# gwall-ceres/HighRes-net

Hardware: AMD Instinct MI355X
Metric: SR frames/sec (384x384 out) at B=32, n_views=32 (higher is better)
Workload: dtype bf16

## Files before the change

### highres-net_amd/hrnet_hip/csrc/api.hip

```cpp
#include "../../../include/hrnet_hip.h"
#include "kernels.h"
#include "hrnet_layout.h"
#include "shiftnet_layout.h"

#include <stdarg.h>
#include <stdio.h>
#include <stdlib.h>
#include <string.h>

static thread_local char g_err[512] = "";
void hrn_set_error(const char* fmt, ...) {
    va_list ap;
    va_start(ap, fmt);
    vsnprintf(g_err, sizeof g_err, fmt, ap);
    va_end(ap);
}

namespace {

using namespace hrn;

struct HrnetWs {
    size_t ref, emb, buf_a, buf_b, fused, total;
};
HrnetWs hrnet_ws(int dt, int B, int V, int H, int W) {
    HrnetWs w;
    const size_t es = hrn_esize(dt), hw = (size_t)H * W;
    const size_t stack = (size_t)B * V * hw * 64 * es;
    size_t off = 0;
    auto take = [&](size_t bytes) { size_t o = off; off = hrn_align_up(off + bytes, ALIGN); return o; };
    w.ref = take((size_t)B * hw * 4);
    w.emb = take(stack);
    w.buf_a = take(stack);
    w.buf_b = take(stack);
    w.fused = take((size_t)B * hw * 64 * es);
    w.total = off;
    return w;
}

size_t stack_lo(int dt, int B, int V, int H, int W) { return dt == HRN_BF16X3 ? (size_t)B * V * H * W * 64 * 2 : 0; }
size_t fused_lo(int dt, int B, int H, int W) { return dt == HRN_BF16X3 ? (size_t)B * H * W * 64 * 2 : 0; }
bool dtype_ok(int dt) { return dt == HRN_F32 || dt == HRN_BF16 || dt == HRN_BF16X3; }

int check_scale(int scale) {
    HRN_CHECK(hrn_scale_ok(scale), -2, "scale must be 2, 3 or 4 (decoder kernel_size == stride; got %d)", scale);
    return 0;
}

int check_common(int dt, int nl, int B, int V, int H, int W) {
    HRN_CHECK(dtype_ok(dt), -2, "dtype must be HRN_DTYPE_F32, HRN_DTYPE_BF16 or HRN_DTYPE_BF16X3 (got %d)", dt);
    HRN_CHECK(nl >= 0 && nl <= HRN_MAX_RES_LAYERS, -2, "num_layers %d out of range 0..%d", nl, HRN_MAX_RES_LAYERS);
    HRN_CHECK(B > 0 && V > 0 && H > 0 && W > 0, -2, "empty input B=%d V=%d H=%d W=%d", B, V, H, W);
    return 0;
}

int encoder_impl(const void* pk, int dt, int nl, const float* lrs, int B, int V, int H, int W,
                 void* emb, void* ws, const HrnetWs& wl, hipStream_t s) {
    const HrnetLayout L = hrnet_layout(dt, nl, 3);
    const size_t hw = (size_t)H * W;
    float* ref = (float*)at(ws, wl.ref);
    void* bufA = at(ws, wl.buf_a);
    void* bufB = at(ws, wl.buf_b);
    int rc;
    if ((rc = hrn_launch_median(lrs, ref, B, V, H, W, s))) return rc;
    const size_t lo = stack_lo(dt, B, V, H, W);
    if ((rc = hrn_launch_stem(dt, lrs, hw, ref, V, hw, nullptr, (const float*)at(pk, L.stem_w), (const float*)at(pk, L.stem_b),
                              (const float*)at(pk, L.stem_a), bufA, B * V, H, W, s, lo))) return rc;
    for (int l = 0; l < nl; ++l) {
        ConvParams p = conv_base(B * V, H, W);
        p.in = bufA; p.out = bufB; p.in_lo = p.out_lo = lo;
        p.wpk = at(pk, L.enc_w[2 * l]); p.bias = (const float*)at(pk, L.enc_b[2 * l]); p.slope = (const float*)at(pk, L.enc_a[2 * l]);
        if ((rc = hrn_launch_conv3x3(dt, 64, 64, p, s, false))) return rc;
        ConvParams q = conv_base(B * V, H, W);
        q.in = bufB; q.out = bufA; q.res = bufA; q.res_mode = 1; q.in_lo = q.out_lo = q.res_lo = lo;
        q.wpk = at(pk, L.enc_w[2 * l + 1]); q.bias = (const float*)at(pk, L.enc_b[2 * l + 1]); q.slope = (const float*)at(pk, L.enc_a[2 * l + 1]);
        if ((rc = hrn_launch_conv3x3(dt, 64, 64, q, s, false))) return rc;
    }
    ConvParams f = conv_base(B * V, H, W);
    f.in = bufA; f.out = emb; f.in_lo = f.out_lo = lo;
    f.wpk = at(pk, L.encf_w); f.bias = (const float*)at(pk, L.encf_b); f.slope = nullptr;
    return hrn_launch_conv3x3(dt, 64, 64, f, s, false);
}

int fuse_impl(const void* pk, int dt, int nl, int alpha_residual, void* emb, const float* alphas, int B, int V, int H, int W,
              void* fused, void* ws, const HrnetWs& wl, hipStream_t s) {
    const HrnetLayout L = hrnet_layout(dt, nl, 3);
    const size_t hw = (size_t)H * W, es = hrn_esize(dt);
    void* t1 = at(ws, wl.buf_a);
    void* t2 = at(ws, wl.buf_b);
    const size_t lo = stack_lo(dt, B, V, H, W), flo = fused_lo(dt, B, H, W);
    int n = V, rc;
    if (n / 2 == 0) {
        HRN_HIP(hipMemcpyAsync(fused, emb, (size_t)B * hw * 64 * es, hipMemcpyDeviceToDevice, s));
        return 0;
    }
    while (n / 2 > 0) {
        const int parity = n & 1, half = n >> 1;
        const bool last = (half == 1);
        ConvParams a = conv_base(B * half, H, W);
        a.in_pair = 1; a.stack = emb; a.pair_h = half; a.pair_last = n - parity - 1; a.pair_vs = V;
        a.out = t1; a.stack_lo = a.out_lo = lo;
        a.wpk = at(pk, L.fres_w[0]); a.bias = (const float*)at(pk, L.fres_b[0]); a.slope = (const float*)at(pk, L.fres_a[0]);
        if ((rc = hrn_launch_conv3x3(dt, 128, 128, a, s, false))) return rc;
        ConvParams b = conv_base(B * half, H, W);
        b.in = t1; b.out = t2; b.in_lo = b.out_lo = b.stack_lo = lo;
        b.res_mode = 2;
        b.stack = emb; b.pair_h = half; b.pair_last = n - parity - 1; b.pair_vs = V;
        b.wpk = at(pk, L.fres_w[1]); b.bias = (const float*)at(pk, L.fres_b[1]); b.slope = (const float*)at(pk, L.fres_a[1]);
        if ((rc = hrn_launch_conv3x3(dt, 128, 128, b, s, false))) return rc;
        ConvParams c = conv_base(B * half, H, W);
        c.in = t2; c.in_lo = c.res_lo = lo;
        c.out_h = half;
        if (last) { c.out = fused; c.out_vs = 1; c.out_lo = flo; } else { c.out = emb; c.out_vs = V; c.out_lo = lo; }
        c.pair_last = n - parity - 1;
        if (alpha_residual) { c.res_mode = 3; c.res = emb; c.res_vs = V; c.alphas = alphas; c.alpha_vs = V; }
        c.wpk = at(pk, L.fout_w); c.bias = (const float*)at(pk, L.fout_b); c.slope = (const float*)at(pk, L.fout_a);
        if ((rc = hrn_launch_conv3x3(dt, 128, 64, c, s, false))) return rc;
        n = half;
    }
    return 0;
}

int decoder_impl(const void* pk, int dt, int nl, int scale, const void* fused, int N, int H, int W, float* sr, hipStream_t s) {
    const HrnetLayout L = hrnet_layout(dt, nl, scale);
    return hrn_launch_decoder(dt, fused, at(pk, L.dec_w), (const float*)at(pk, L.dec_b), (const float*)at(pk, L.dec_a),
                              (const float*)at(pk, L.fin_w), (const float*)at(pk, L.fin_b), sr, N, H, W, s, fused_lo(dt, N, H, W), scale);
}

struct SnWs {
    size_t means, scale, shift, partial, x, y, fc, xr, fc_partial, total;
};
SnWs sn_ws(int B) {
    SnWs w;
    size_t off = 0;
    auto take = [&](size_t bytes) { size_t o = off; off = hrn_align_up(off + bytes, ALIGN); return o; };
    w.means = take((size_t)B * 2 * 4);
    w.scale = take(128 * 4); w.shift = take(128 * 4);
    w.partial = take((size_t)SN_PARTIAL_BLOCKS * 128 * 2 * 8);
    w.x = take((size_t)B * 128 * 128 * 64 * 4);
    w.y = take((size_t)B * 128 * 128 * 64 * 4);
    w.fc = take((size_t)B * 1024 * 4);
    w.xr = take((size_t)B * 32768 * 4);
    w.fc_partial = take(hrn_fc1_partial_bytes());
    w.total = off;
    return w;
}

}

extern "C" {

int hrn_version(void) { return HRN_ABI_VERSION; }
const char* hrn_last_error(void) { return g_err; }

size_t hrn_hrnet_packed_bytes_s(int dtype, int num_layers, int scale) {
    if (!dtype_ok(dtype) || num_layers < 0 || num_layers > HRN_MAX_RES_LAYERS || !hrn_scale_ok(scale)) return 0;
    return hrnet_layout(dtype, num_layers, scale).total;
}

int hrn_hrnet_pack_s(const hrn_hrnet_params* P, int dt, int scale, void* packed, size_t packed_bytes, void* stream) {
    int rc;
    if ((rc = check_scale(scale))) return rc;
    HRN_CHECK(P && packed, -2, "hrn_hrnet_pack: null argument");
    if ((rc = check_common(dt, P->num_layers, 1, 1, 1, 1))) return rc;
    const int nl = P->num_layers;
    const HrnetLayout L = hrnet_layout(dt, nl, scale);
    HRN_CHECK(packed_bytes >= L.total, -3, "hrn_hrnet_pack: packed buffer too small (%zu < %zu)", packed_bytes, L.total);
    hipStream_t s = (hipStream_t)stream;
    auto copy = [&](size_t off, const float* src, size_t n) -> int {
        HRN_CHECK(src != nullptr, -2, "hrn_hrnet_pack: null parameter pointer");
        HRN_HIP(hipMemcpyAsync(at(packed, off), src, n * 4, hipMemcpyDeviceToDevice, s));
        return 0;
    };
    if ((rc = copy(L.stem_w, P->enc_init_w, 64 * 18)) || (rc = copy(L.stem_b, P->enc_init_b, 64)) || (rc = copy(L.stem_a, P->enc_init_a, 1))) return rc;
    for (int i = 0; i < 2 * nl; ++i) {
        HRN_CHECK(P->enc_res_w[i], -2, "hrn_hrnet_pack: null encoder weight %d", i);
        if ((rc = hrn_launch_conv_pack(dt, 64, 64, P->enc_res_w[i], at(packed, L.enc_w[i]), s))) return rc;
        if ((rc = copy(L.enc_b[i], P->enc_res_b[i], 64)) || (rc = copy(L.enc_a[i], P->enc_res_a[i], 1))) return rc;
    }
    HRN_CHECK(P->enc_final_w && P->fuse_out_w && P->dec_w, -2, "hrn_hrnet_pack: null weight pointer");
    if ((rc = hrn_launch_conv_pack(dt, 64, 64, P->enc_final_w, at(packed, L.encf_w), s))) return rc;
    if ((rc = copy(L.encf_b, P->enc_final_b, 64))) return rc;
    for (int i = 0; i < 2; ++i) {
        HRN_CHECK(P->fuse_res_w[i], -2, "hrn_hrnet_pack: null fuse weight %d", i);
        if ((rc = hrn_launch_conv_pack(dt, 128, 128, P->fuse_res_w[i], at(packed, L.fres_w[i]), s))) return rc;
        if ((rc = copy(L.fres_b[i], P->fuse_res_b[i], 128)) || (rc = copy(L.fres_a[i], P->fuse_res_a[i], 1))) return rc;
    }
    if ((rc = hrn_launch_conv_pack(dt, 128, 64, P->fuse_out_w, at(packed, L.fout_w), s))) return rc;
    if ((rc = copy(L.fout_b, P->fuse_out_b, 64)) || (rc = copy(L.fout_a, P->fuse_out_a, 1))) return rc;
    if ((rc = hrn_launch_decoder_pack(dt == HRN_BF16X3 ? HRN_F32 : dt, P->dec_w, at(packed, L.dec_w), s, scale))) return rc;
    if ((rc = copy(L.dec_b, P->dec_b, 64)) || (rc = copy(L.dec_a, P->dec_a, 1))) return rc;
    if ((rc = copy(L.fin_w, P->fin_w, 64)) || (rc = copy(L.fin_b, P->fin_b, 1))) return rc;
    return 0;
}

size_t hrn_hrnet_workspace_bytes(int dtype, int B, int V, int H, int W) {
    if (!dtype_ok(dtype) || B <= 0 || V <= 0 || H <= 0 || W <= 0) return 0;
    return hrnet_ws(dtype, B, V, H, W).total;
}

int hrn_encoder_forward(const void* packed, int dt, int nl, const float* lrs, int B, int V, int H, int W,
                        void* emb, void* ws, size_t ws_bytes, void* stream) {
    int rc;
    if ((rc = check_common(dt, nl, B, V, H, W))) return rc;
    HRN_CHECK(packed && lrs && emb && ws, -2, "hrn_encoder_forward: null argument");
    const HrnetWs wl = hrnet_ws(dt, B, V, H, W);
    HRN_CHECK(ws_bytes >= wl.total, -3, "hrn_encoder_forward: workspace too small (%zu < %zu)", ws_bytes, wl.total);
    return encoder_impl(packed, dt, nl, lrs, B, V, H, W, emb, ws, wl, (hipStream_t)stream);
}

int hrn_fuse_forward(const void* packed, int dt, int nl, int alpha_residual, void* emb, const float* alphas,
                     int B, int V, int H, int W, void* fused, void* ws, size_t ws_bytes, void* stream) {
    int rc;
    if ((rc = check_common(dt, nl, B, V, H, W))) return rc;
    HRN_CHECK(packed && emb && alphas && fused && ws, -2, "hrn_fuse_forward: null argument");
    const HrnetWs wl = hrnet_ws(dt, B, V, H, W);
    HRN_CHECK(ws_bytes >= wl.total, -3, "hrn_fuse_forward: workspace too small (%zu < %zu)", ws_bytes, wl.total);
    return fuse_impl(packed, dt, nl, alpha_residual, emb, alphas, B, V, H, W, fused, ws, wl, (hipStream_t)stream);
}

int hrn_decoder_forward_s(const void* packed, int dt, int nl, int scale, const void* fused, int N, int H, int W, float* sr, void* stream) {
    int rc;
    if ((rc = check_scale(scale)) || (rc = check_common(dt, nl, N, 1, H, W))) return rc;
    HRN_CHECK(packed && fused && sr, -2, "hrn_decoder_forward: null argument");
    return decoder_impl(packed, dt, nl, scale, fused, N, H, W, sr, (hipStream_t)stream);
}

int hrn_hrnet_forward_s(const void* packed, int dt, int nl, int scale, int alpha_residual, const float* lrs, const float* alphas,
                        int B, int V, int H, int W, float* sr, void* ws, size_t ws_bytes, void* stream) {
    int rc;
    if ((rc = check_scale(scale)) || (rc = check_common(dt, nl, B, V, H, W))) return rc;
    HRN_CHECK(packed && lrs && alphas && sr && ws, -2, "hrn_hrnet_forward: null argument");
    const HrnetWs wl = hrnet_ws(dt, B, V, H, W);
    HRN_CHECK(ws_bytes >= wl.total, -3, "hrn_hrnet_forward: workspace too small (%zu < %zu)", ws_bytes, wl.total);
    hipStream_t s = (hipStream_t)stream;
    void* emb = at(ws, wl.emb);
    void* fused = at(ws, wl.fused);
    if ((rc = encoder_impl(packed, dt, nl, lrs, B, V, H, W, emb, ws, wl, s))) return rc;
    if ((rc = fuse_impl(packed, dt, nl, alpha_residual, emb, alphas, B, V, H, W, fused, ws, wl, s))) return rc;
    return decoder_impl(packed, dt, nl, scale, fused, B, H, W, sr, s);
}

size_t hrn_shiftnet_packed_bytes(void) { return sn_layout().total; }

int hrn_shiftnet_pack(const hrn_shiftnet_params* P, void* packed, size_t packed_bytes, void* stream) {
    HRN_CHECK(P && packed, -2, "hrn_shiftnet_pack: null argument");
    const SnLayout L = sn_layout();
    HRN_CHECK(packed_bytes >= L.total, -3, "hrn_shiftnet_pack: packed buffer too small (%zu < %zu)", packed_bytes, L.total);
    hipStream_t s = (hipStream_t)stream;
    int rc;
    for (int i = 0; i < 8; ++i) {
        HRN_CHECK(P->conv_w[i] && P->conv_b[i], -2, "hrn_shiftnet_pack: null conv parameter %d", i);
        if (i == 0) {
            HRN_HIP(hipMemcpyAsync(at(packed, L.conv_w[0]), P->conv_w[0], 64 * 18 * 4, hipMemcpyDeviceToDevice, s));
        } else if ((rc = hrn_launch_conv_pack(HRN_F32, SN_CI[i], SN_CO[i], P->conv_w[i], at(packed, L.conv_w[i]), s))) {
            return rc;
        }
        HRN_HIP(hipMemcpyAsync(at(packed, L.conv_b[i]), P->conv_b[i], SN_CO[i] * 4, hipMemcpyDeviceToDevice, s));
    }
    HRN_CHECK(P->fc1_b && P->fc2_w, -2, "hrn_shiftnet_pack: null fc parameter");
    HRN_HIP(hipMemcpyAsync(at(packed, L.fc1_b), P->fc1_b, 1024 * 4, hipMemcpyDeviceToDevice, s));
    HRN_HIP(hipMemcpyAsync(at(packed, L.fc2_w), P->fc2_w, 2 * 1024 * 4, hipMemcpyDeviceToDevice, s));
    return 0;
}

size_t hrn_shiftnet_workspace_bytes(int B) { return B > 0 ? sn_ws(B).total : 0; }

int hrn_shiftnet_forward(const void* packed, const hrn_shiftnet_params* P, const float* x, int B, int train_bn, float momentum,
                         const unsigned char* dropout_mask, float* theta, void* ws, size_t ws_bytes, void* stream) {
    HRN_CHECK(packed && P && x && theta && ws, -2, "hrn_shiftnet_forward: null argument");
    HRN_CHECK(P->fc1_w, -2, "hrn_shiftnet_forward: params->fc1_w is null (fc1.weight is read in place)");
    HRN_CHECK(B > 0, -2, "hrn_shiftnet_forward: empty batch");
    const SnLayout L = sn_layout();
    const SnWs wl = sn_ws(B);
    HRN_CHECK(ws_bytes >= wl.total, -3, "hrn_shiftnet_forward: workspace too small (%zu < %zu)", ws_bytes, wl.total);
    hipStream_t s = (hipStream_t)stream;
    float* means = (float*)at(ws, wl.means);
    float* scale = (float*)at(ws, wl.scale);
    float* shift = (float*)at(ws, wl.shift);
    double* partial = (double*)at(ws, wl.partial);
    float* bx = (float*)at(ws, wl.x);
    float* by = (float*)at(ws, wl.y);
    float* fc = (float*)at(ws, wl.fc);
    int rc, hsz = 128;
    const size_t plane = 128 * 128;
    if ((rc = hrn_launch_plane_mean(x, means, B * 2, plane, s))) return rc;
    for (int i = 0; i < 8; ++i) {
        HRN_CHECK(P->bn_g[i] && P->bn_b[i] && P->bn_rm[i] && P->bn_rv[i], -2, "hrn_shiftnet_forward: null BatchNorm tensor %d", i);
        const int C = SN_CO[i];
        if (i > 0 && !train_bn) {
            if ((rc = hrn_launch_bn_fold(P->bn_g[i], P->bn_b[i], P->bn_rm[i], P->bn_rv[i], 1e-5f, (const float*)at(packed, L.conv_b[i]),
                                         scale, shift, C, s))) return rc;
            ConvParams p = conv_base(B, hsz, hsz);
            p.in = by; p.out = bx;
            p.wpk = at(packed, L.conv_w[i]); p.scale = scale; p.bias = shift; p.relu = 1;
            if ((rc = hrn_launch_conv3x3(HRN_F32, SN_CI[i], C, p, s, false))) return rc;
            if (SN_POOL[i]) {
                if ((rc = hrn_launch_bn_act_pool(HRN_F32, bx, nullptr, nullptr, by, B, hsz, hsz, C, 1, s))) return rc;
                hsz /= 2;
            } else {
                float* t = bx; bx = by; by = t;
            }
            continue;
        }
        if (i == 0) {
            if ((rc = hrn_launch_stem(HRN_F32, x, 2 * plane, x + plane, 1, 2 * plane, means, (const float*)at(packed, L.conv_w[0]),
                                      (const float*)at(packed, L.conv_b[0]), nullptr, bx, B, hsz, hsz, s, 0))) return rc;
        } else {
            ConvParams p = conv_base(B, hsz, hsz);
            p.in = by; p.out = bx;
            p.wpk = at(packed, L.conv_w[i]); p.bias = (const float*)at(packed, L.conv_b[i]);
            if ((rc = hrn_launch_conv3x3(HRN_F32, SN_CI[i], SN_CO[i], p, s, false))) return rc;
        }
        if (train_bn) {
            if ((rc = hrn_launch_bn_stats(HRN_F32, bx, (size_t)B * hsz * hsz, C, P->bn_g[i], P->bn_b[i], 1e-5f, scale, shift,
                                          P->bn_rm[i], P->bn_rv[i], momentum, partial, SN_PARTIAL_BLOCKS, s))) return rc;
        } else {
            if ((rc = hrn_launch_bn_fold(P->bn_g[i], P->bn_b[i], P->bn_rm[i], P->bn_rv[i], 1e-5f, nullptr, scale, shift, C, s))) return rc;
        }
        if ((rc = hrn_launch_bn_act_pool(HRN_F32, bx, scale, shift, by, B, hsz, hsz, C, SN_POOL[i], s))) return rc;
        if (SN_POOL[i]) hsz /= 2;
    }
    float* xr = (float*)at(ws, wl.xr);
    if ((rc = hrn_launch_fc_to_ref(HRN_F32, by, dropout_mask, xr, B, s))) return rc;
    if ((rc = hrn_launch_fc1(xr, P->fc1_w, (const float*)at(packed, L.fc1_b), fc, B, (float*)at(ws, wl.fc_partial), s))) return rc;
    return hrn_launch_fc2(fc, (const float*)at(packed, L.fc2_w), theta, B, s);
}

int hrn_lanczos_kernel(const float* dx, int n, float* taps, void* stream) {
    HRN_CHECK(n >= 0 && (n == 0 || (dx && taps)), -2, "hrn_lanczos_kernel: bad argument");
    return hrn_launch_lanczos_taps(dx, n, taps, (hipStream_t)stream);
}

int hrn_lanczos_shift(const float* img, const float* shift, int b, int c, int H, int W, float* out, void* stream) {
    HRN_CHECK(b >= 0 && c >= 0 && H > 0 && W > 0, -2, "hrn_lanczos_shift: bad shape");
    HRN_CHECK(b * c == 0 || (img && shift && out), -2, "hrn_lanczos_shift: null argument");
    return hrn_launch_lanczos_shift(img, shift, b, c, H, W, out, (hipStream_t)stream);
}

size_t hrn_lanczos_shift_backward_workspace_bytes(int b, int c, int H, int W) {
    if (b <= 0 || c <= 0 || H <= 0 || W <= 0) return 0;
    return hrn_lanczos_bwd_workspace_bytes_impl(b, c, H, W);
}

int hrn_lanczos_shift_backward(const float* img, const float* shift, const float* d_out, int b, int c, int H, int W, float* d_img,
                               float* d_shift, void* ws, size_t ws_bytes, void* stream) {
    HRN_CHECK(img && shift && d_out && ws, -2, "hrn_lanczos_shift_backward: null argument");
    HRN_CHECK(b > 0 && c > 0, -2, "hrn_lanczos_shift_backward: empty input b=%d c=%d", b, c);
    HRN_CHECK(ws_bytes >= hrn_lanczos_bwd_workspace_bytes_impl(b, c, H, W), -3, "hrn_lanczos_shift_backward: workspace too small");
    return hrn_launch_lanczos_shift_bwd(img, shift, d_out, b, c, H, W, d_img, d_shift, ws, (hipStream_t)stream);
}

int hrn_get_loss(const float* srs, const float* hrs, const float* maps, int B, int S, int crop, int metric, float* out, void* stream) {
    HRN_CHECK(B > 0 && S > 0 && crop >= 0 && 2 * crop < S, -2, "hrn_get_loss: bad shape B=%d S=%d crop=%d", B, S, crop);
    HRN_CHECK(metric >= 0 && metric <= 2, -2, "hrn_get_loss: metric must be 0 (masked_MSE), 1 (cMSE) or 2 (cPSNR)");
    HRN_CHECK(srs && hrs && maps && out, -2, "hrn_get_loss: null argument");
    return hrn_launch_masked_cmse(srs, hrs, maps, B, S, crop, metric, out, (hipStream_t)stream);
}

size_t hrn_get_loss_train_workspace_bytes(int B) { return B > 0 ? hrn_loss_train_workspace_bytes_impl(B) : 0; }

int hrn_get_loss_train(const float* srs, const float* hrs, const float* maps, int B, int S, int crop, int metric, float* out,
                       double* stats, void* ws, size_t ws_bytes, void* stream) {
    HRN_CHECK(B > 0 && B <= 65535 && S > 0 && crop >= 0 && 2 * crop < S, -2, "hrn_get_loss_train: bad shape B=%d S=%d crop=%d", B, S, crop);
    HRN_CHECK(metric == 1 || metric == 2, -2, "hrn_get_loss_train: metric must be 1 (cMSE) or 2 (cPSNR); masked_MSE has no registered form");
    HRN_CHECK(srs && hrs && maps && out && stats && ws, -2, "hrn_get_loss_train: null argument");
    HRN_CHECK(ws_bytes >= hrn_loss_train_workspace_bytes_impl(B), -3, "hrn_get_loss_train: workspace too small");
    return hrn_launch_loss_train(srs, hrs, maps, B, S, crop, metric, out, stats, (double*)ws, (hipStream_t)stream);
}

int hrn_get_loss_backward(const float* srs, const float* hrs, const float* maps, const double* stats, const float* d_out, int B, int S,
                          int crop, int metric, float* d_srs, void* stream) {
    HRN_CHECK(B > 0 && B <= 65535 && S > 0 && crop >= 0 && 2 * crop < S, -2, "hrn_get_loss_backward: bad shape B=%d S=%d crop=%d", B, S, crop);
    HRN_CHECK(metric == 1 || metric == 2, -2, "hrn_get_loss_backward: metric must be 1 (cMSE) or 2 (cPSNR)");
    HRN_CHECK(srs && hrs && maps && stats && d_out && d_srs, -2, "hrn_get_loss_backward: null argument");
    return hrn_launch_loss_backward(srs, hrs, maps, stats, d_out, B, S, crop, metric, d_srs, (hipStream_t)stream);
}

size_t hrn_shift_cpsnr_workspace_bytes(int B, int border) {
    if (B <= 0 || border < 0) return 0;
    return (size_t)B * (2 * border + 1) * (2 * border + 1) * sizeof(double);
}

int hrn_shift_cpsnr(const float* srs, const float* hrs, const float* maps, int B, int S, int border, int clip, float* out,
                    void* ws, size_t ws_bytes, void* stream) {
    HRN_CHECK(B > 0 && border >= 0 && S > 2 * border, -2, "hrn_shift_cpsnr: bad shape B=%d S=%d border=%d", B, S, border);
    HRN_CHECK(B <= 65535, -2, "hrn_shift_cpsnr: batch %d exceeds the grid limit", B);
    HRN_CHECK(srs && hrs && maps && out && ws, -2, "hrn_shift_cpsnr: null argument");
    HRN_CHECK(ws_bytes >= hrn_shift_cpsnr_workspace_bytes(B, border), -3, "hrn_shift_cpsnr: workspace too small");
    return hrn_launch_shift_cpsnr(srs, hrs, maps, B, S, border, clip, (double*)ws, out, (hipStream_t)stream);
}

}
```

### highres-net_amd/hrnet_hip/csrc/conv3x3.h

```cpp
#pragma once
#include "common.h"

#define CONV_TILE_H 8
#define CONV_TILE_W 32
#define CONV_STEP_BYTES 8192

struct ConvParams {
    const void* in;
    const void* stack;
    int in_pair;
    void* out;
    const void* res;
    const float* alphas;
    const void* wpk;
    const float* bias;
    const float* slope;
    int M, H, W;
    int pair_h, pair_last, pair_vs;
    int out_h, out_vs;
    int res_mode;
    int alpha_vs, res_vs;
    int relu;
    const float* scale;
    size_t in_lo, stack_lo, out_lo, res_lo;
    const float* only_if_nonpos;
};

static inline size_t conv_packed_elems(int cin, int cout) { return (size_t)cin * cout * 9; }

int hrn_launch_conv3x3(int dt, int cin, int cout, const ConvParams& p, hipStream_t stream, bool general_only);

int hrn_launch_conv3x3_r64(const ConvParams& p, hipStream_t stream);

int hrn_launch_conv3x3_v6(int cin, int cout, const ConvParams& p, hipStream_t stream);

int hrn_launch_conv3x3_v6x3(int cin, int cout, const ConvParams& p, hipStream_t stream);

int hrn_launch_conv_pack(int dt, int cin, int cout, const float* w_oihw, void* packed, hipStream_t stream);
```

### highres-net_amd/hrnet_hip/csrc/conv3x3.hip

```cpp
#include "conv3x3.h"
#include <stdlib.h>


namespace {

constexpr int HALO_H = CONV_TILE_H + 2;
constexpr int HALO_W = CONV_TILE_W + 2;
constexpr int PIX_PITCH = 144;
constexpr int IN_LDS_BYTES = HALO_H * HALO_W * PIX_PITCH;
constexpr int W_ROW_PITCH = 144;
constexpr int N_IN_CHUNKS16 = HALO_H * HALO_W * 8;

struct TileCtx {
    int m, y0, x0;
    const unsigned char* src0;
    const unsigned char* src1;
    const unsigned char* in_plain;
};

template <int DT, int CIN, int COUT>
__global__ __launch_bounds__(256 * (COUT / 64), 2) void conv3x3_kernel(const ConvParams p) {
    extern __shared__ __attribute__((aligned(16))) unsigned char smem[];
    unsigned char* in_lds = smem;
    unsigned char* w_lds = smem + IN_LDS_BYTES;

    constexpr int ES = ElemOf<DT>::size;
    constexpr int KB = 128 / ES;
    constexpr int NCHUNK = CIN / KB;
    constexpr int NHALF = COUT / 64;
    constexpr int NT = 256 * NHALF;
    constexpr int NSTEP = NCHUNK * 9;
    constexpr int W_BUF_BYTES = COUT * W_ROW_PITCH;
    constexpr int N_IN_ITERS = (N_IN_CHUNKS16 + NT - 1) / NT;

    if (p.only_if_nonpos && p.only_if_nonpos[0] > 0.f) return;
    const int tid = threadIdx.x;
    const int lane = tid & 63, wave = (tid >> 6) & 3, half = tid >> 8;
    const int r = lane & 31, hh = lane >> 5;
    const int H = p.H, W = p.W;
    const size_t hw = (size_t)H * W;
    const int tiles_x = (W + CONV_TILE_W - 1) / CONV_TILE_W;
    const int tiles_y = (H + CONV_TILE_H - 1) / CONV_TILE_H;
    const int tiles = tiles_x * tiles_y;
    const long total = (long)tiles * p.M;

    const int G = gridDim.x;
    const int bid = blockIdx.x;
    const int slot = (G & 7) == 0 ? (bid & 7) * (G >> 3) + (bid >> 3) : bid;
    long tile = slot;
    if (tile >= total) return;

    const bool in_pair = p.in_pair != 0;
    const int in_pix_bytes = in_pair ? 64 * ES : CIN * ES;

    auto make_tile = [&](long tl) {
        TileCtx c;
        c.m = (int)(tl / tiles);
        const int t = (int)(tl - (long)c.m * tiles);
        const int ty = t / tiles_x;
        c.y0 = ty * CONV_TILE_H;
        c.x0 = (t - ty * tiles_x) * CONV_TILE_W;
        c.src0 = c.src1 = nullptr;
        if (p.pair_h > 0) {
            const int b = c.m / p.pair_h, i = c.m - b * p.pair_h;
            c.src0 = (const unsigned char*)p.stack + ((size_t)b * p.pair_vs + i) * hw * 64 * ES;
            c.src1 = (const unsigned char*)p.stack + ((size_t)b * p.pair_vs + (p.pair_last - i)) * hw * 64 * ES;
        }
        c.in_plain = (const unsigned char*)p.in + (size_t)c.m * hw * CIN * ES;
        return c;
    };

    uint4 inreg[N_IN_ITERS];
    auto issue_input = [&](const TileCtx& c, int chunk) {
        const unsigned char* base;
        int choff;
        if (in_pair) {
            const int ch0 = chunk * KB;
            base = ch0 < 64 ? c.src0 : c.src1;
            choff = (ch0 & 63) * ES;
        } else {
            base = c.in_plain;
            choff = chunk * 128;
        }
#pragma unroll
        for (int it = 0; it < N_IN_ITERS; ++it) {
            const int cc = tid + it * NT;
            const int pix = cc >> 3, part = cc & 7;
            const int py = pix / HALO_W, px = pix - py * HALO_W;
            const int gy = c.y0 + py - 1, gx = c.x0 + px - 1;
            uint4 v = make_uint4(0u, 0u, 0u, 0u);
            if (cc < N_IN_CHUNKS16 && (unsigned)gy < (unsigned)H && (unsigned)gx < (unsigned)W)
                v = *(const uint4*)(base + ((size_t)gy * W + gx) * in_pix_bytes + choff + part * 16);
            inreg[it] = v;
        }
    };
    auto commit_input = [&]() {
#pragma unroll
        for (int it = 0; it < N_IN_ITERS; ++it) {
            const int cc = tid + it * NT;
            if (cc < N_IN_CHUNKS16) *(uint4*)(in_lds + (cc >> 3) * PIX_PITCH + (cc & 7) * 16) = inreg[it];
        }
    };

    const uint4* wg = (const uint4*)p.wpk;
    const int w_dst0 = (tid >> 3) * W_ROW_PITCH + (tid & 7) * 16;
    const int w_dst1 = w_dst0 + (NT / 8) * W_ROW_PITCH;
    const unsigned char* a_base = w_lds + (half * 64 + r) * W_ROW_PITCH + hh * 16;
    const unsigned char* b_base = in_lds + ((2 * wave) * HALO_W + r) * PIX_PITCH + hh * 16;

    const bool has_slope = p.slope != nullptr;
    const float slope = has_slope ? p.slope[0] : 0.f;

    TileCtx cur = make_tile(tile);
    issue_input(cur, 0);
    commit_input();
    {
        const uint4 w0 = wg[tid], w1 = wg[tid + NT];
        *(uint4*)(w_lds + w_dst0) = w0;
        *(uint4*)(w_lds + w_dst1) = w1;
    }
    __syncthreads();

    int gstep = 0;
    for (;;) {
        const long ntile = tile + G;
        const bool has_next_tile = ntile < total;
        const TileCtx nxt = has_next_tile ? make_tile(ntile) : cur;

        f32x16 acc[2][2];
#pragma unroll
        for (int a = 0; a < 2; ++a)
#pragma unroll
            for (int b = 0; b < 2; ++b)
#pragma unroll
                for (int e = 0; e < 16; ++e) acc[a][b][e] = 0.f;

#pragma unroll 1
        for (int chunk = 0; chunk < NCHUNK; ++chunk) {
            const bool last_chunk = chunk == NCHUNK - 1;
            const bool has_next = !last_chunk || has_next_tile;
            if (has_next) {
                if (last_chunk) issue_input(nxt, 0); else issue_input(cur, chunk + 1);
                __builtin_amdgcn_sched_barrier(0);
            }
#pragma unroll
            for (int tap = 0; tap < 9; ++tap) {
                const int ky = tap / 3, kx = tap - ky * 3;
                const unsigned char* xb = b_base + (ky * HALO_W + kx) * PIX_PITCH;
                {
                    const int s = chunk * 9 + tap;
                    const bool last_step = s == NSTEP - 1;
                    const bool more = !last_step || has_next_tile;
                    uint4 w0, w1;
                    if (more) {
                        const size_t ns = last_step ? 0 : (size_t)(s + 1);
                        w0 = wg[ns * (2 * NT) + tid];
                        w1 = wg[ns * (2 * NT) + tid + NT];
                        __builtin_amdgcn_sched_barrier(0);
                    }
                    const unsigned char* wb = a_base + (gstep & 1) * W_BUF_BYTES;
                    if constexpr (DT == HRN_BF16) {
                        constexpr int KBATCH = NT == 512 ? 4 : 2;
#pragma unroll
                        for (int k0 = 0; k0 < 4; k0 += KBATCH) {
                            bf16x8 a0[KBATCH], a1[KBATCH], b0[KBATCH], b1[KBATCH];
#pragma unroll
                            for (int ks = 0; ks < KBATCH; ++ks) {
                                a0[ks] = *(const bf16x8*)(wb + (k0 + ks) * 32);
                                b0[ks] = *(const bf16x8*)(xb + (k0 + ks) * 32);
                                a1[ks] = *(const bf16x8*)(wb + 32 * W_ROW_PITCH + (k0 + ks) * 32);
                                b1[ks] = *(const bf16x8*)(xb + HALO_W * PIX_PITCH + (k0 + ks) * 32);
                            }
                            __builtin_amdgcn_sched_barrier(0);
#pragma unroll
                            for (int ks = 0; ks < KBATCH; ++ks) {
                                acc[0][0] = __builtin_amdgcn_mfma_f32_32x32x16_bf16(a0[ks], b0[ks], acc[0][0], 0, 0, 0);
                                acc[0][1] = __builtin_amdgcn_mfma_f32_32x32x16_bf16(a1[ks], b0[ks], acc[0][1], 0, 0, 0);
                                acc[1][0] = __builtin_amdgcn_mfma_f32_32x32x16_bf16(a0[ks], b1[ks], acc[1][0], 0, 0, 0);
                                acc[1][1] = __builtin_amdgcn_mfma_f32_32x32x16_bf16(a1[ks], b1[ks], acc[1][1], 0, 0, 0);
                            }
                        }
                    } else {
#pragma unroll
                        for (int q = 0; q < 4; ++q) {
                            const f32x4 a0 = *(const f32x4*)(wb + q * 32);
                            const f32x4 a1 = *(const f32x4*)(wb + 32 * W_ROW_PITCH + q * 32);
                            const f32x4 b0 = *(const f32x4*)(xb + q * 32);
                            const f32x4 b1 = *(const f32x4*)(xb + HALO_W * PIX_PITCH + q * 32);
#pragma unroll
                            for (int j = 0; j < 4; ++j) {
                                acc[0][0] = __builtin_amdgcn_mfma_f32_32x32x2f32(a0[j], b0[j], acc[0][0], 0, 0, 0);
                                acc[0][1] = __builtin_amdgcn_mfma_f32_32x32x2f32(a1[j], b0[j], acc[0][1], 0, 0, 0);
                                acc[1][0] = __builtin_amdgcn_mfma_f32_32x32x2f32(a0[j], b1[j], acc[1][0], 0, 0, 0);
                                acc[1][1] = __builtin_amdgcn_mfma_f32_32x32x2f32(a1[j], b1[j], acc[1][1], 0, 0, 0);
                            }
                        }
                    }
                    if (more) {
                        unsigned char* wd = w_lds + ((gstep + 1) & 1) * W_BUF_BYTES;
                        *(uint4*)(wd + w_dst0) = w0;
                        *(uint4*)(wd + w_dst1) = w1;
                    }
                    __syncthreads();
                    ++gstep;
                }
            }
            if (has_next) commit_input();
            if (!last_chunk) __syncthreads();
        }

        {
            const int m = cur.m;
            size_t out_img;
            float alpha = 1.f;
            const unsigned char* res3 = nullptr;
            if (p.out_h > 0) {
                const int b = m / p.out_h, i = m - b * p.out_h;
                out_img = (size_t)b * p.out_vs + i;
                if (p.res_mode == 3) {
                    if (p.alphas) alpha = p.alphas[(size_t)b * p.alpha_vs + (p.pair_last - i)];
                    res3 = (const unsigned char*)p.res + ((size_t)b * p.res_vs + i) * hw * COUT * ES;
                }
            } else {
                out_img = (size_t)m;
            }
            unsigned char* outp = (unsigned char*)p.out + out_img * hw * COUT * ES;
            const int gx = cur.x0 + r;
#pragma unroll
            for (int pb = 0; pb < 2; ++pb) {
                const int gy = cur.y0 + 2 * wave + pb;
                if (gy >= H || gx >= W) continue;
                const size_t pix = (size_t)gy * W + gx;
                {
#pragma unroll
                    for (int cb = 0; cb < 2; ++cb) {
#pragma unroll
                        for (int g = 0; g < 4; ++g) {
                            const int co = half * 64 + cb * 32 + 8 * g + 4 * hh;
                            f32x4 v;
#pragma unroll
                            for (int j = 0; j < 4; ++j) v[j] = acc[pb][cb][4 * g + j];
                            if (p.scale) {
                                const f32x4 sc = *(const f32x4*)(p.scale + co);
                                v *= sc;
                            }
                            v += *(const f32x4*)(p.bias + co);
                            if (has_slope) {
#pragma unroll
                                for (int j = 0; j < 4; ++j) v[j] = v[j] >= 0.f ? v[j] : slope * v[j];
                            }
                            if (p.relu) {
#pragma unroll
                                for (int j = 0; j < 4; ++j) v[j] = fmaxf(v[j], 0.f);
                            }
                            if (p.res_mode == 1) {
                                v += load4<DT>((const unsigned char*)p.res + (size_t)m * hw * COUT * ES, pix * COUT + co);
                            } else if (p.res_mode == 2) {
                                v += load4<DT>(half == 0 ? cur.src0 : cur.src1, pix * 64 + (co & 63));
                            } else if (p.res_mode == 3) {
                                v = load4<DT>(res3, pix * COUT + co) + alpha * v;
                            }
                            store4<DT>(outp, pix * COUT + co, v);
                        }
                    }
                }
            }
        }
        if (!has_next_tile) break;
        __syncthreads();
        tile = ntile;
        cur = nxt;
    }
}


template <int DT, int CIN, int COUT>
int launch(const ConvParams& p, hipStream_t stream) {
    constexpr int LDS_BYTES = IN_LDS_BYTES + 2 * COUT * W_ROW_PITCH;
    { const int rc_lds = hrn_allow_lds((const void*)conv3x3_kernel<DT, CIN, COUT>, LDS_BYTES); if (rc_lds) return rc_lds; }
    const long tiles = (long)((p.W + CONV_TILE_W - 1) / CONV_TILE_W) * ((p.H + CONV_TILE_H - 1) / CONV_TILE_H);
    const long total = tiles * p.M;
    HRN_CHECK(total > 0 && total < (1L << 40), -2, "conv3x3: bad tile count %ld", total);
    long grid = (2L / (COUT / 64)) * hrn_device_cus();
    if (total < grid) grid = total;
    if (grid >= 8) grid &= ~7L;
    static const char* fam_names[2][2][2] = {{{"conv3x3_f32_64x64", "conv3x3_f32_64x128"}, {"conv3x3_f32_128x64", "conv3x3_f32_128x128"}},
                                             {{"conv3x3_bf16_64x64", "conv3x3_bf16_64x128"}, {"conv3x3_bf16_128x64", "conv3x3_bf16_128x128"}}};
    const double px = (double)p.M * p.H * p.W, es = ElemOf<DT>::size;
    HrnProfScope prof(fam_names[DT][CIN / 128][COUT / 128], 2.0 * CIN * COUT * 9 * px,
                      px * es * (CIN + COUT + (p.res_mode ? COUT : 0)), stream);
    hipLaunchKernelGGL((conv3x3_kernel<DT, CIN, COUT>), dim3((unsigned)grid), dim3(256 * (COUT / 64)), LDS_BYTES, stream, p);
    HRN_LAUNCH_CHECK();
    return 0;
}

template <int DT>
__global__ void conv_pack_kernel(const float* __restrict__ w, void* __restrict__ out, int cin, int cout) {
    constexpr int ES = ElemOf<DT>::size;
    constexpr int KB = 128 / ES;
    const int nhalf = cout / 64;
    const size_t total = (size_t)cin * cout * 9;
    for (size_t idx = (size_t)blockIdx.x * blockDim.x + threadIdx.x; idx < total; idx += (size_t)gridDim.x * blockDim.x) {
        const int kk = (int)(idx % KB);
        const int col = (int)((idx / KB) % 64);
        const int step = (int)(idx / ((size_t)KB * 64));
        const int half = step % nhalf;
        const int ct = step / nhalf;
        const int tap = ct % 9, chunk = ct / 9;
        const int co = half * 64 + col, ci = chunk * KB + kk;
        const float v = w[((size_t)co * cin + ci) * 9 + tap];
        store_elem<DT>(out, idx, v);
    }
}

__global__ void conv_pack_x3_kernel(const float* __restrict__ w, unsigned short* __restrict__ out, int cin, int cout) {
    constexpr int KB = 64;
    const int nhalf = cout / 64;
    const size_t total = (size_t)cin * cout * 9;
    for (size_t idx = (size_t)blockIdx.x * blockDim.x + threadIdx.x; idx < total; idx += (size_t)gridDim.x * blockDim.x) {
        const int kk = (int)(idx % KB);
        const int col = (int)((idx / KB) % 64);
        const int step = (int)(idx / ((size_t)KB * 64));
        const int half = step % nhalf;
        const int ct = step / nhalf;
        const int tap = ct % 9, chunk = ct / 9;
        const int co = half * 64 + col, ci = chunk * KB + kk;
        const float v = w[((size_t)co * cin + ci) * 9 + tap];
        const unsigned short h = f32_to_bf16_bits(v);
        out[idx] = h;
        out[total + idx] = f32_to_bf16_bits(v - bf16_bits_to_f32(h));
    }
}

}

int hrn_launch_conv3x3(int dt, int cin, int cout, const ConvParams& p, hipStream_t stream, bool general_only) {
    HRN_CHECK(p.M > 0 && p.H > 0 && p.W > 0, -2, "conv3x3: empty problem M=%d H=%d W=%d", p.M, p.H, p.W);
    HRN_CHECK(!p.in_pair || (cin == 128 && p.pair_h > 0 && p.stack), -2, "conv3x3: pair input needs cin=128 and a pair descriptor");
    HRN_CHECK(p.res_mode != 2 || (p.pair_h > 0 && p.stack && cout == 128), -2, "conv3x3: res_mode 2 needs a pair descriptor and cout=128");
    HRN_CHECK(p.in_pair || p.in, -2, "conv3x3: null input");
    HRN_CHECK(p.res_mode != 3 || p.out_h > 0, -2, "conv3x3: res_mode 3 needs slot output");
    HRN_CHECK(!(general_only && dt == HRN_BF16X3), -2, "conv3x3: bf16x3 has no general kernel");
    if (dt == HRN_BF16X3) return hrn_launch_conv3x3_v6x3(cin, cout, p, stream);
    if (dt == HRN_BF16 && !p.scale && !p.relu && !general_only) {
        static const int r64 = [] { const char* e = getenv("HRN_CONV_R64"); return e ? atoi(e) : 1; }();
        static const int v6 = [] { const char* e = getenv("HRN_CONV_V6"); return e ? atoi(e) : 1; }();
        if (cin == 64 && cout == 64 && r64) { const int rc = hrn_launch_conv3x3_r64(p, stream); if (rc != -100) return rc; }
        if ((cin == 128 || cout == 128) && v6) { const int rc = hrn_launch_conv3x3_v6(cin, cout, p, stream); if (rc != -100) return rc; }
    }
#define HRN_CONV_CASE(DT_, CI_, CO_) if (dt == DT_ && cin == CI_ && cout == CO_) return launch<DT_, CI_, CO_>(p, stream);
    HRN_CONV_CASE(HRN_BF16, 64, 64)
    HRN_CONV_CASE(HRN_BF16, 64, 128)
    HRN_CONV_CASE(HRN_BF16, 128, 64)
    HRN_CONV_CASE(HRN_BF16, 128, 128)
    HRN_CONV_CASE(HRN_F32, 64, 64)
    HRN_CONV_CASE(HRN_F32, 64, 128)
    HRN_CONV_CASE(HRN_F32, 128, 64)
    HRN_CONV_CASE(HRN_F32, 128, 128)
#undef HRN_CONV_CASE
    hrn_set_error("conv3x3: unsupported dtype/channels dt=%d cin=%d cout=%d", dt, cin, cout);
    return -2;
}

int hrn_launch_conv_pack(int dt, int cin, int cout, const float* w, void* packed, hipStream_t stream) {
    HRN_CHECK((cin == 64 || cin == 128) && (cout == 64 || cout == 128), -2, "conv pack: unsupported channels %d->%d", cin, cout);
    const size_t total = (size_t)cin * cout * 9;
    const int blocks = (int)((total + 255) / 256 < 1024 ? (total + 255) / 256 : 1024);
    if (dt == HRN_BF16X3) hipLaunchKernelGGL(conv_pack_x3_kernel, dim3(blocks), dim3(256), 0, stream, w, (unsigned short*)packed, cin, cout);
    else if (dt == HRN_BF16) hipLaunchKernelGGL(conv_pack_kernel<HRN_BF16>, dim3(blocks), dim3(256), 0, stream, w, packed, cin, cout);
    else hipLaunchKernelGGL(conv_pack_kernel<HRN_F32>, dim3(blocks), dim3(256), 0, stream, w, packed, cin, cout);
    HRN_LAUNCH_CHECK();
    return 0;
}
```

### highres-net_amd/hrnet_hip/csrc/conv3x3_r64.hip

```cpp
#include <type_traits>
#include "conv3x3.h"

namespace {

constexpr int HALO_H = CONV_TILE_H + 2;
constexpr int HALO_W = CONV_TILE_W + 2;
constexpr int IN_BYTES = HALO_H * HALO_W * 128;
constexpr int W_BYTES = 9 * 64 * 128;
constexpr int LDS_BYTES = W_BYTES + 2 * IN_BYTES + 256;

__device__ __forceinline__ void lds_done_then_barrier() {
    asm volatile("s_waitcnt lgkmcnt(0)" ::: "memory");
    __builtin_amdgcn_s_barrier();
    asm volatile("" ::: "memory");
}

__device__ __forceinline__ float raw_max(float a, float b) {
    float y;
    asm("v_max_f32 %0, %1, %2" : "=v"(y) : "v"(a), "v"(b));
    return y;
}

__device__ __attribute__((aligned(16))) unsigned hrn_r64_zero16[4];

template <bool RES>
__global__ __launch_bounds__(512, 2) void conv3x3_r64_kernel(const ConvParams p) {
    if (p.only_if_nonpos && p.only_if_nonpos[0] > 0.f) return;
    extern __shared__ __attribute__((aligned(16))) unsigned char smem[];
    unsigned char* w_lds = smem;
    float* bias_lds = (float*)(smem + W_BYTES + 2 * IN_BYTES);

    const int tid = threadIdx.x;
    const int lane = tid & 63;
    const int wave = __builtin_amdgcn_readfirstlane(tid >> 6);
    const int team = wave >> 2, tw = wave & 3;
    unsigned char* in_lds = smem + W_BYTES + team * IN_BYTES;
    const int r = lane & 31, hh = lane >> 5;
    const int H = p.H, W = p.W;
    const size_t hw = (size_t)H * W;
    const unsigned tiles_x = (W + CONV_TILE_W - 1) / CONV_TILE_W;
    const unsigned tiles_y = (H + CONV_TILE_H - 1) / CONV_TILE_H;
    const unsigned tiles = tiles_x * tiles_y;
    const unsigned total = tiles * (unsigned)p.M;
    const unsigned G = gridDim.x;
    const unsigned bid = blockIdx.x;
    const unsigned slot = (G & 7) == 0 ? (bid & 7) * (G >> 3) + (bid >> 3) : bid;
    if (slot >= total) return;
    const int ntl = (int)((total - slot + G - 1) / G);
    const int nmine = (ntl + 1 - team) >> 1;

    unsigned cur_m = (slot + team * G) / tiles, cur_t = (slot + team * G) - cur_m * tiles;
    const unsigned step_m = (2 * G) / tiles, step_t = 2 * G - step_m * tiles;

    {
        const u32x4* wg = (const u32x4*)p.wpk;
#pragma unroll
        for (int j = 0; j < W_BYTES / 16 / 512; ++j) {
            const int idx = tid + j * 512;
            const int row = idx >> 3, c = idx & 7;
            *(u32x4*)(w_lds + row * 128 + ((c ^ ((row >> 1) & 7)) << 4)) = wg[idx];
        }
        if (tid < 64) bias_lds[tid] = p.bias[tid];
    }

    unsigned voff[11], cm_lo = 0, cm_hi = 0;
    if (!RES) {
#pragma unroll
        for (int jj = 0; jj < 11; ++jj) {
            const int j = tw + 4 * jj;
            const int pix = j * 8 + (lane >> 3);
            const int py = pix / HALO_W, px = pix - py * HALO_W;
            voff[jj] = (unsigned)((py * W + px) * 128 + (((lane & 7) ^ ((pix >> 1) & 7)) << 4));
            unsigned cls = (py == 0 ? 1u : 0u) | (py == HALO_H - 1 ? 2u : 0u) | (px == 0 ? 4u : 0u) | (px == HALO_W - 1 ? 8u : 0u);
            if (pix >= HALO_H * HALO_W) cls = 0;
            if (jj < 8) cm_lo |= cls << (4 * jj); else cm_hi |= cls << (4 * (jj - 8));
        }
    }
    unsigned pend_F = 0;
    auto issue = [&](unsigned m, unsigned t) __attribute__((always_inline)) {
        const int ty = t / tiles_x;
        const int y0 = ty * CONV_TILE_H, x0 = (t - ty * tiles_x) * CONV_TILE_W;
        const unsigned char* base = (const unsigned char*)p.in + (size_t)m * hw * 128;
        const bool fast = !RES && y0 + CONV_TILE_H <= H && x0 + CONV_TILE_W <= W && (m > 0 || y0 > 0) &&
                          ((int)m + 1 < p.M || (size_t)(y0 + CONV_TILE_H) * W + x0 + CONV_TILE_W < hw);
        pend_F = 0;
        if (fast) {
            const unsigned char* hb = base + ((long)(y0 - 1) * W + (x0 - 1)) * 128;
#pragma unroll
            for (int jj = 0; jj < 11; ++jj) {
                const int j = tw + 4 * jj;
                if (j < 43) {
                    if (jj < 10 || j * 8 + (lane >> 3) < HALO_H * HALO_W)
                        __builtin_amdgcn_global_load_lds((const __attribute__((address_space(1))) void*)(hb + voff[jj]),
                                                         (__attribute__((address_space(3))) void*)(in_lds + j * 1024), 16, 0, 0);
                }
            }
            pend_F = (y0 == 0 ? 1u : 0u) | (y0 + CONV_TILE_H == H ? 2u : 0u) | (x0 == 0 ? 4u : 0u) | (x0 + CONV_TILE_W == W ? 8u : 0u);
            __builtin_amdgcn_sched_barrier(0);
            return;
        }
        int lq = lane;
        asm volatile("" : "+v"(lq));
#pragma unroll
        for (int jj = 0; jj < 11; ++jj) {
            const int j = tw + 4 * jj;
            if (j < 43) {
                const int pix = j * 8 + (lq >> 3);
                const int lc = (lq & 7) ^ ((pix >> 1) & 7);
                const int py = pix / HALO_W, px = pix - py * HALO_W;
                const int gy = y0 - 1 + py, gx = x0 - 1 + px;
                const bool ok = (unsigned)gy < (unsigned)H && (unsigned)gx < (unsigned)W;
                const unsigned char* src = ok ? base + (unsigned)((gy * W + gx) * 128 + lc * 16) : (const unsigned char*)hrn_r64_zero16;
                if (pix < HALO_H * HALO_W)
                    __builtin_amdgcn_global_load_lds((const __attribute__((address_space(1))) void*)src,
                                                     (__attribute__((address_space(3))) void*)(in_lds + j * 1024), 16, 0, 0);
            }
        }
        __builtin_amdgcn_sched_barrier(0);
    };
    auto fix_borders = [&]() __attribute__((always_inline)) {
        if (!RES && pend_F) {
            const unsigned fm = pend_F * 0x11111111u;
            const unsigned hit_lo = cm_lo & fm, hit_hi = cm_hi & fm;
            const u32x4 z = {0u, 0u, 0u, 0u};
#pragma unroll
            for (int jj = 0; jj < 11; ++jj) {
                const int j = tw + 4 * jj;
                if (j < 43) {
                    const unsigned h = jj < 8 ? (hit_lo >> (4 * jj)) & 15u : (hit_hi >> (4 * (jj - 8))) & 15u;
                    if (h) *(u32x4*)(in_lds + j * 1024 + lane * 16) = z;
                }
            }
        }
    };

    const bool has_slope = p.slope != nullptr;
    const float slope = has_slope ? p.slope[0] : 0.f;
    const bool slope01 = slope >= 0.f && slope <= 1.f;
    const unsigned lds0 = (unsigned)(__UINTPTR_TYPE__)(__attribute__((address_space(3))) unsigned char*)smem;
    unsigned a_off[4], a_off_hi[4], b_off[4][3];
#pragma unroll
    for (int ks = 0; ks < 4; ++ks) {
        a_off[ks] = lds0 + r * 128 + (((ks * 2 + hh) ^ ((r >> 1) & 7)) << 4);
        a_off_hi[ks] = a_off[ks] + 4 * 8192;
    }
#pragma unroll
    for (int row = 0; row < 4; ++row)
#pragma unroll
        for (int kx = 0; kx < 3; ++kx) {
            const int pix = (2 * tw + row) * HALO_W + r + kx;
            b_off[row][kx] = lds0 + (unsigned)(W_BYTES + team * IN_BYTES) + (((unsigned)pix << 7) | ((unsigned)(((pix >> 1) & 7) ^ hh) << 4));
        }

    f32x16 acc[2][2];

    auto multiply = [&]() __attribute__((always_inline)) {
#pragma unroll
        for (int cb = 0; cb < 2; ++cb)
#pragma unroll
            for (int g = 0; g < 4; ++g) {
                const f32x4 b = *(const f32x4*)(bias_lds + cb * 32 + 8 * g + 4 * hh);
#pragma unroll
                for (int j = 0; j < 4; ++j) { acc[cb][0][4 * g + j] = b[j]; acc[cb][1][4 * g + j] = b[j]; }
            }
        constexpr int NK = 36;
        bf16x8 fa[3][2], fb[3][2];
        auto rd = [&](bf16x8& dst, unsigned addr, int imm) __attribute__((always_inline)) {
            asm volatile("ds_read_b128 %0, %1 offset:%2" : "=v"(dst) : "v"(addr), "n"(imm));
        };
        auto load_part = [&](int i, int part) __attribute__((always_inline)) {
            const int s_ = i % 3, tap = i >> 2, ks = i & 3;
            const int ky = tap / 3, kx = tap - ky * 3;
            if (part < 2) {
                rd(fa[s_][part], tap < 4 ? a_off[ks] : a_off_hi[ks], (tap < 4 ? tap : tap - 4) * 8192 + part * 4096);
            } else {
                unsigned kbits = 0;
                if (ks) asm volatile("s_mov_b32 %0, %1" : "=s"(kbits) : "n"(ks << 5));
                rd(fb[s_][part - 2], b_off[part - 2 + ky][kx] ^ kbits, 0);
            }
        };
        asm volatile("s_waitcnt lgkmcnt(0)" ::: "memory");
        __builtin_amdgcn_s_setprio(3);
#pragma unroll
        for (int i = 0; i < 2; ++i)
#pragma unroll
            for (int part = 0; part < 4; ++part) load_part(i, part);
        __builtin_amdgcn_sched_barrier(0);
#pragma unroll
        for (int i = 0; i < NK; ++i) {
            const int s_ = i % 3;
            const bool more = i + 2 < NK;
            if (i < NK - 1) asm volatile("s_waitcnt lgkmcnt(5)" : "+v"(fa[s_][0]), "+v"(fb[s_][0]));
            else asm volatile("s_waitcnt lgkmcnt(1)" : "+v"(fa[s_][0]), "+v"(fb[s_][0]));
            acc[0][0] = __builtin_amdgcn_mfma_f32_32x32x16_bf16(fa[s_][0], fb[s_][0], acc[0][0], 0, 0, 0);
            if (more) load_part(i + 2, 0);
            __builtin_amdgcn_sched_barrier(0);
            if (more) asm volatile("s_waitcnt lgkmcnt(5)" : "+v"(fb[s_][1]));
            else if (i == NK - 2) asm volatile("s_waitcnt lgkmcnt(4)" : "+v"(fb[s_][1]));
            else asm volatile("s_waitcnt lgkmcnt(0)" : "+v"(fb[s_][1]));
            acc[0][1] = __builtin_amdgcn_mfma_f32_32x32x16_bf16(fa[s_][0], fb[s_][1], acc[0][1], 0, 0, 0);
            if (more) load_part(i + 2, 1);
            __builtin_amdgcn_sched_barrier(0);
            asm volatile("" : "+v"(fa[s_][1]));
            acc[1][0] = __builtin_amdgcn_mfma_f32_32x32x16_bf16(fa[s_][1], fb[s_][0], acc[1][0], 0, 0, 0);
            if (more) load_part(i + 2, 2);
            __builtin_amdgcn_sched_barrier(0);
            acc[1][1] = __builtin_amdgcn_mfma_f32_32x32x16_bf16(fa[s_][1], fb[s_][1], acc[1][1], 0, 0, 0);
            if (more) load_part(i + 2, 3);
            __builtin_amdgcn_sched_barrier(0);
        }
        __builtin_amdgcn_s_setprio(0);
    };

    u32x4 resv[2][4];
    float res_alpha = 1.f;
    auto fetch_residual = [&]() __attribute__((always_inline)) {
        const int m = (int)cur_m;
        const int ty = cur_t / tiles_x;
        const int y0 = ty * CONV_TILE_H, x0 = (cur_t - ty * tiles_x) * CONV_TILE_W;
        const unsigned char* rbase = (const unsigned char*)p.res + (size_t)m * hw * 128;
        if (p.res_mode == 3) {
            const int ob = m / p.out_h, oi = m - ob * p.out_h;
            rbase = (const unsigned char*)p.res + ((size_t)ob * p.res_vs + oi) * hw * 128;
            res_alpha = p.alphas ? p.alphas[(size_t)ob * p.alpha_vs + (p.pair_last - oi)] : 1.f;
        }
#pragma unroll
        for (int pb = 0; pb < 2; ++pb) {
            const int gy = y0 + 2 * tw + pb, gyc = gy < H ? gy : H - 1;
#pragma unroll
            for (int j = 0; j < 4; ++j) {
                const int gxj = x0 + (r & ~3) + j, gxjc = gxj < W ? gxj : W - 1;
                resv[pb][j] = __builtin_nontemporal_load((const u32x4*)(rbase + (unsigned)((gyc * W + gxjc) * 128 + hh * 64 + (r & 3) * 16)));
            }
        }
    };

    auto finish = [&](bool more) __attribute__((always_inline)) {
        const int m = (int)cur_m;
        const int ty = cur_t / tiles_x;
        const int y0 = ty * CONV_TILE_H, x0 = (cur_t - ty * tiles_x) * CONV_TILE_W;
        cur_t += step_t; cur_m += step_m;
        if (cur_t >= tiles) { cur_t -= tiles; ++cur_m; }
        size_t oimg = (size_t)m;
        int ob = 0, oi = 0;
        if (p.out_h > 0) { ob = m / p.out_h; oi = m - ob * p.out_h; oimg = (size_t)ob * p.out_vs + oi; }
        unsigned char* outp = (unsigned char*)p.out + (oimg * hw + (size_t)y0 * W + x0) * 128;
        if (RES) {
#pragma unroll
            for (int pb = 0; pb < 2; ++pb)
#pragma unroll
                for (int g = 0; g < 4; ++g) asm volatile("" :: "v"(resv[pb][g]));
            asm volatile("" :: "v"(res_alpha));
        }
        if (more) issue(cur_m, cur_t);
        auto epilogue = [&](auto act_c) __attribute__((always_inline)) {
        constexpr int ACT = decltype(act_c)::value;
#pragma unroll
        for (int pb = 0; pb < 2; ++pb) {
            const int gy = y0 + 2 * tw + pb;
            u32x4 uu[4];
            if (RES) quad_transpose(resv[pb], (lane & 1) != 0, (lane & 2) != 0);
#pragma unroll
            for (int g = 0; g < 4; ++g) {
                float xa[4], xb[4];
#pragma unroll
                for (int j = 0; j < 4; ++j) { xa[j] = acc[0][pb][4 * g + j]; xb[j] = acc[1][pb][4 * g + j]; }
                if (ACT == 1) {
#pragma unroll
                    for (int j = 0; j < 4; ++j) { xa[j] = raw_max(xa[j], slope * xa[j]); xb[j] = raw_max(xb[j], slope * xb[j]); }
                } else if (ACT == 2) {
#pragma unroll
                    for (int j = 0; j < 4; ++j) { xa[j] = xa[j] >= 0.f ? xa[j] : slope * xa[j]; xb[j] = xb[j] >= 0.f ? xb[j] : slope * xb[j]; }
                }
                u32x4 u;
                if (RES) {
                    float v[8];
#pragma unroll
                    for (int j = 0; j < 4; ++j) {
                        const u32x2 sw = __builtin_amdgcn_permlane32_swap(__float_as_uint(xa[j]), __float_as_uint(xb[j]), false, false);
                        v[j] = __uint_as_float(sw[0]);
                        v[4 + j] = __uint_as_float(sw[1]);
                    }
                    const u32x4 rq = resv[pb][g];
#pragma unroll
                    for (int j = 0; j < 4; ++j) {
                        const float r0 = __uint_as_float(rq[j] << 16), r1 = __uint_as_float(rq[j] & 0xffff0000u);
                        if (p.res_mode == 3) { v[2 * j] = r0 + res_alpha * v[2 * j]; v[2 * j + 1] = r1 + res_alpha * v[2 * j + 1]; }
                        else { v[2 * j] += r0; v[2 * j + 1] += r1; }
                    }
#pragma unroll
                    for (int j = 0; j < 4; ++j) u[j] = pack2_bf16(v[2 * j], v[2 * j + 1]);
                } else {
                    const u32x2 s0 = __builtin_amdgcn_permlane32_swap(pack2_bf16(xa[0], xa[1]), pack2_bf16(xb[0], xb[1]), false, false);
                    const u32x2 s1 = __builtin_amdgcn_permlane32_swap(pack2_bf16(xa[2], xa[3]), pack2_bf16(xb[2], xb[3]), false, false);
                    u[0] = s0[0]; u[1] = s1[0]; u[2] = s0[1]; u[3] = s1[1];
                }
                uu[g] = u;
            }
            {
                quad_transpose(uu, (lane & 1) != 0, (lane & 2) != 0);
                unsigned char* oq = outp + (unsigned)(((2 * tw + pb) * W + (r & ~3)) * 128 + hh * 64 + (r & 3) * 16);
#pragma unroll
                for (int j = 0; j < 4; ++j)
                    if (gy < H && x0 + (r & ~3) + j < W) __builtin_nontemporal_store(uu[j], (u32x4*)(oq + j * 128));
            }
        }
        };
        if (!has_slope) epilogue(std::integral_constant<int, 0>{});
        else if (slope01) epilogue(std::integral_constant<int, 1>{});
        else epilogue(std::integral_constant<int, 2>{});
        {
            const int nst = 4 * ((y0 + 2 * tw < H) + (y0 + 2 * tw + 1 < H));
            if (nst == 8) asm volatile("s_waitcnt vmcnt(8)" ::: "memory");
            else if (nst == 4) asm volatile("s_waitcnt vmcnt(4)" ::: "memory");
            else asm volatile("s_waitcnt vmcnt(0)" ::: "memory");
        }
        fix_borders();
    };

    if (nmine > 0) issue(cur_m, cur_t);
    asm volatile("s_waitcnt vmcnt(0)" ::: "memory");
    fix_borders();
    lds_done_then_barrier();

    for (int ph = 0; ph <= ntl; ++ph) {
        const int q = ph - team;
        if (q >= 0) {
            const int k = q >> 1;
            if (k < nmine) {
                if ((q & 1) == 0) { if (RES) fetch_residual(); multiply(); }
                else finish(k + 1 < nmine);
            }
        }
        if (ph < ntl) lds_done_then_barrier();
    }
}


template <bool RES>
int launch_r64(const ConvParams& p, long grid, hipStream_t stream) {
    { const int rc_lds = hrn_allow_lds((const void*)conv3x3_r64_kernel<RES>, LDS_BYTES); if (rc_lds) return rc_lds; }
    hipLaunchKernelGGL(conv3x3_r64_kernel<RES>, dim3((unsigned)grid), dim3(512), LDS_BYTES, stream, p);
    HRN_LAUNCH_CHECK();
    return 0;
}

}

int hrn_launch_conv3x3_r64(const ConvParams& p, hipStream_t stream) {
    if (p.scale || p.relu || p.in_pair || p.res_mode == 2) return -100;
    static_assert(LDS_BYTES <= 160 * 1024, "LDS budget");
    const long tiles = (long)((p.W + CONV_TILE_W - 1) / CONV_TILE_W) * ((p.H + CONV_TILE_H - 1) / CONV_TILE_H);
    const long total = tiles * p.M;
    HRN_CHECK(total > 0, -2, "conv3x3_r64: bad tile count %ld", total);
    if (total >= (1L << 30) || (long)p.H * p.W * 128 >= (1L << 31)) return -100;
    long grid = hrn_device_cus();
    if (total < grid) grid = total;
    if (grid >= 8) grid &= ~7L;
    const double px = (double)p.M * p.H * p.W;
    HrnProfScope prof(p.res_mode ? "conv3x3_bf16_64x64+res" : "conv3x3_bf16_64x64", 2.0 * 64 * 64 * 9 * px,
                      px * 2 * (64 + 64 + (p.res_mode ? 64 : 0)), stream);
    return p.res_mode ? launch_r64<true>(p, grid, stream) : launch_r64<false>(p, grid, stream);
}
```

### highres-net_amd/hrnet_hip/csrc/kernels.h

```cpp
#pragma once
#include "common.h"
#include "conv3x3.h"

int hrn_launch_median(const float* lrs, float* ref, int B, int V, int H, int W, hipStream_t stream);
int hrn_launch_stem(int dt, const float* in0, size_t img_stride0, const float* in1, int rep1, size_t img_stride1,
                    const float* sub, const float* w, const float* bias, const float* slope, void* out,
                    int M, int H, int W, hipStream_t stream, size_t out_lo);
int hrn_launch_planes_to_f32(const void* hi, size_t lo_off, float* out, size_t n, hipStream_t stream);
int hrn_launch_f32_to_planes(const float* in, void* hi, size_t lo_off, size_t n, hipStream_t stream);
int hrn_launch_stem_pre(int dt, const float* in0, size_t img_stride0, const float* in1, int rep1, size_t img_stride1, const float* w,
                        const float* bias, void* out, int M, int H, int W, const float* only_if_nonpos, hipStream_t stream);
int hrn_launch_plane_mean(const float* x, float* mean, int planes, size_t hw, hipStream_t stream);

int hrn_launch_decoder(int dt, const void* fused, const void* wpk, const float* bias, const float* slope,
                       const float* wf, const float* bf, float* sr, int N, int H, int W, hipStream_t stream, size_t fused_lo, int scale);
int hrn_launch_decoder_pack(int dt, const float* w_iokk, void* packed, hipStream_t stream, int scale);

int hrn_launch_lanczos_taps(const float* d, int n, float* taps, hipStream_t stream);
int hrn_launch_lanczos_shift(const float* img, const float* shift, int b, int c, int H, int W, float* out, hipStream_t stream);
size_t hrn_lanczos_bwd_workspace_bytes_impl(int b, int c, int H, int W);
int hrn_launch_lanczos_shift_bwd(const float* img, const float* shift, const float* dout, int b, int c, int H, int W, float* d_img,
                                 float* d_shift, void* ws, hipStream_t stream);

int hrn_launch_masked_cmse(const float* srs, const float* hrs, const float* maps, int B, int S, int crop, int metric, float* out,
                           hipStream_t stream);
size_t hrn_loss_train_workspace_bytes_impl(int B);
int hrn_launch_loss_train(const float* srs, const float* hrs, const float* maps, int B, int S, int crop, int metric, float* out,
                          double* stats, double* partial, hipStream_t stream);
int hrn_launch_loss_backward(const float* srs, const float* hrs, const float* maps, const double* stats, const float* d_out, int B,
                             int S, int crop, int metric, float* d_srs, hipStream_t stream);
int hrn_launch_shift_cpsnr(const float* srs, const float* hrs, const float* maps, int B, int S, int border, int clip,
                           double* scores, float* out, hipStream_t stream);

int hrn_launch_bn_stats(int dt, const void* x, size_t npix, int C, const float* gamma, const float* beta, float eps,
                        float* scale, float* shift, float* running_mean, float* running_var, float momentum,
                        double* partial, int partial_blocks, hipStream_t stream);
int hrn_launch_bn_fold(const float* gamma, const float* beta, const float* rm, const float* rv, float eps,
                       const float* conv_bias, float* scale, float* shift, int C, hipStream_t stream);
int hrn_launch_bn_act_pool(int dt, const void* x, const float* scale, const float* shift, void* out, int N, int H, int W, int C,
                           int pool, hipStream_t stream);
int hrn_launch_fc_to_ref(int dt, const void* y, const unsigned char* mask, float* xr, int B, hipStream_t stream);
size_t hrn_fc1_partial_bytes(void);
int hrn_launch_fc1(const float* xr, const float* w, const float* b, float* y, int B, float* partial, hipStream_t stream);
int hrn_launch_fc2(const float* y, const float* w, float* theta, int B, hipStream_t stream);
int hrn_launch_sn_bn_bwd(int dt, const void* x, const void* dy, const float* stats, const float* gamma, void* dx, float* dgamma, float* dbeta,
                         int N, int H, int W, int C, int pool, double* partial, double* sums, hipStream_t s);
int hrn_launch_sn_stem_dgrad(int dt, const void* g, const float* w, float* din, int M, int H, int W, hipStream_t s);
int hrn_launch_fc_from_ref(int dt, const float* dxr, const unsigned char* mask, void* dy, int B, hipStream_t s);
int hrn_launch_sn_bn_save_stats(const double* partial, size_t npix, int C, float eps, float* mean, float* invstd, hipStream_t s);
int hrn_launch_sn_sub_plane_mean(const float* g, const float* means, float* out, int planes, size_t hw, hipStream_t s);
int hrn_launch_sn_fc2_bwd(const float* dtheta, const float* y1, const float* w2, float* dz1, float* dw2, float* db1, int B, hipStream_t s);
int hrn_launch_sn_fc1_bwd_w(const float* dz1, const float* xr, float* dw1, int B, hipStream_t s);
int hrn_launch_sn_fc1_bwd_x(const float* dz1, const float* w1, float* dxr, int B, hipStream_t s);
```

### highres-net_amd/hrnet_hip/csrc/stem.hip

```cpp
#include "kernels.h"

namespace {

__device__ __forceinline__ void cswap(float& a, float& b) {
    const float lo = fminf(a, b), hi = fmaxf(a, b);
    a = lo; b = hi;
}

__global__ void median_kernel(const float* __restrict__ lrs, float* __restrict__ ref, int V, size_t hw, size_t total) {
    const int n = V < 9 ? V : 9;
    for (size_t idx = (size_t)blockIdx.x * blockDim.x + threadIdx.x; idx < total; idx += (size_t)gridDim.x * blockDim.x) {
        const size_t b = idx / hw, pix = idx - b * hw;
        const float* src = lrs + b * V * hw + pix;
        float v[9];
#pragma unroll
        for (int i = 0; i < 9; ++i) v[i] = i < n ? src[(size_t)i * hw] : __builtin_inff();
        cswap(v[0], v[3]); cswap(v[1], v[7]); cswap(v[2], v[5]); cswap(v[4], v[8]);
        cswap(v[0], v[7]); cswap(v[2], v[4]); cswap(v[3], v[8]); cswap(v[5], v[6]);
        cswap(v[0], v[2]); cswap(v[1], v[3]); cswap(v[4], v[5]); cswap(v[7], v[8]);
        cswap(v[1], v[4]); cswap(v[3], v[6]); cswap(v[5], v[7]);
        cswap(v[0], v[1]); cswap(v[2], v[4]); cswap(v[3], v[5]); cswap(v[6], v[8]);
        cswap(v[2], v[3]); cswap(v[4], v[5]); cswap(v[6], v[7]);
        cswap(v[1], v[2]); cswap(v[3], v[4]); cswap(v[5], v[6]);
        const int k = (n - 1) >> 1;
        float out = v[0];
#pragma unroll
        for (int i = 1; i < 9; ++i) out = (i == k) ? v[i] : out;
        ref[idx] = out;
    }
}

template <int DT>
__global__ __launch_bounds__(256) void stem_kernel(const float* __restrict__ in0, const float* __restrict__ in1,
                                                   size_t img_stride0, int rep1, size_t img_stride1,
                                                   const float* __restrict__ sub,
                                                   const float* __restrict__ w, const float* __restrict__ bias,
                                                   const float* __restrict__ slope, void* __restrict__ out,
                                                   int M, int H, int W, const float* __restrict__ only_if_nonpos, size_t out_lo) {
    if (only_if_nonpos && only_if_nonpos[0] > 0.f) return;
    __shared__ __attribute__((aligned(16))) float wl[18 * 64];
    __shared__ __attribute__((aligned(16))) float bl[64];
    for (int i = threadIdx.x; i < 18 * 64; i += 256) {
        const int co = i & 63, k = i >> 6;
        wl[i] = w[co * 18 + k];
    }
    if (threadIdx.x < 64) bl[threadIdx.x] = bias[threadIdx.x];
    __syncthreads();
    const float a = slope ? slope[0] : 1.f;
    const int cg = threadIdx.x & 7;
    const int xl = threadIdx.x >> 3;
    const int px_tiles = (W + 31) >> 5, py_tiles = (H + 3) >> 2;
    const size_t patches = (size_t)M * py_tiles * px_tiles;
    for (size_t pi = blockIdx.x; pi < patches; pi += gridDim.x) {
        const int tx = (int)(pi % px_tiles);
        const int ty = (int)((pi / px_tiles) % py_tiles);
        const int m = (int)(pi / ((size_t)px_tiles * py_tiles));
        const int x = tx * 32 + xl, y0 = ty * 4;
        const float* p0 = in0 + (size_t)m * img_stride0;
        const float* p1 = in1 + (size_t)(m / rep1) * img_stride1;
        const float s0 = sub ? sub[2 * m] : 0.f, s1 = sub ? sub[2 * m + 1] : 0.f;
        float win[2][6][3];
#pragma unroll
        for (int dy = 0; dy < 6; ++dy) {
            const int gy = y0 + dy - 1;
#pragma unroll
            for (int dx = 0; dx < 3; ++dx) {
                const int gx = x + dx - 1;
                const bool ok = (unsigned)gy < (unsigned)H && (unsigned)gx < (unsigned)W;
                win[0][dy][dx] = ok ? p0[(size_t)gy * W + gx] - s0 : 0.f;
                win[1][dy][dx] = ok ? p1[(size_t)gy * W + gx] - s1 : 0.f;
            }
        }
        float acc[4][8];
#pragma unroll
        for (int py = 0; py < 4; ++py)
#pragma unroll
            for (int c = 0; c < 8; ++c) acc[py][c] = bl[cg * 8 + c];
#pragma unroll
        for (int ci = 0; ci < 2; ++ci)
#pragma unroll
            for (int dy = 0; dy < 3; ++dy)
#pragma unroll
                for (int dx = 0; dx < 3; ++dx) {
                    const float* wr = wl + (ci * 9 + dy * 3 + dx) * 64 + cg * 8;
                    const f32x4 w0 = *(const f32x4*)(wr), w1 = *(const f32x4*)(wr + 4);
#pragma unroll
                    for (int py = 0; py < 4; ++py) {
                        const float xin = win[ci][py + dy][dx];
#pragma unroll
                        for (int j = 0; j < 4; ++j) {
                            acc[py][j] = fmaf(xin, w0[j], acc[py][j]);
                            acc[py][4 + j] = fmaf(xin, w1[j], acc[py][4 + j]);
                        }
                    }
                }
        if (x < W) {
#pragma unroll
            for (int py = 0; py < 4; ++py) {
                if (y0 + py >= H) continue;
                const size_t o = (((size_t)m * H + y0 + py) * W + x) * 64 + cg * 8;
                f32x4 v0, v1;
#pragma unroll
                for (int j = 0; j < 4; ++j) {
                    const float t0 = acc[py][j], t1 = acc[py][4 + j];
                    v0[j] = t0 >= 0.f ? t0 : a * t0;
                    v1[j] = t1 >= 0.f ? t1 : a * t1;
                }
                if constexpr (DT == HRN_BF16X3) {
                    unsigned h[4], l[4];
                    split2_bf16(v0[0], v0[1], h[0], l[0]); split2_bf16(v0[2], v0[3], h[1], l[1]);
                    split2_bf16(v1[0], v1[1], h[2], l[2]); split2_bf16(v1[2], v1[3], h[3], l[3]);
                    const u32x4 uh = {h[0], h[1], h[2], h[3]}, ul = {l[0], l[1], l[2], l[3]};
                    *(u32x4*)((unsigned short*)out + o) = uh;
                    *(u32x4*)((unsigned char*)out + out_lo + o * 2) = ul;
                } else if constexpr (DT == HRN_BF16) {
                    u32x4 u;
                    u[0] = pack2_bf16(v0[0], v0[1]); u[1] = pack2_bf16(v0[2], v0[3]);
                    u[2] = pack2_bf16(v1[0], v1[1]); u[3] = pack2_bf16(v1[2], v1[3]);
                    *(u32x4*)((unsigned short*)out + o) = u;
                } else {
                    *(f32x4*)((float*)out + o) = v0;
                    *(f32x4*)((float*)out + o + 4) = v1;
                }
            }
        }
    }
}

template <bool X3>
__global__ __launch_bounds__(256) void stem_mfma_kernel(const float* __restrict__ in0, const float* __restrict__ in1,
                                                        size_t img_stride0, int rep1, size_t img_stride1,
                                                        const float* __restrict__ w, const float* __restrict__ bias,
                                                        const float* __restrict__ slope, unsigned short* __restrict__ out,
                                                        int M, int H, int W, size_t out_lo) {
    constexpr int SROW = 144;
    constexpr int NK = X3 ? 4 : 3;
    __shared__ __attribute__((aligned(16))) unsigned char stg_all[(X3 ? 2 : 1) * 4 * 32 * SROW];
    const int tid = threadIdx.x, lane = tid & 63;
    const int wave = __builtin_amdgcn_readfirstlane(tid >> 6);
    const int r = lane & 31, hh = lane >> 5;
    const float a = slope ? slope[0] : 1.f;
    unsigned char* stg = stg_all + wave * 32 * SROW;

    bf16x8 wa[2][NK];
#pragma unroll
    for (int cb = 0; cb < 2; ++cb)
#pragma unroll
        for (int s = 0; s < NK; ++s)
#pragma unroll
            for (int j = 0; j < 8; ++j) {
                const int n = 8 * s + j, co = cb * 32 + r;
                float v = 0.f;
                bool want_lo = false;
                if (n < 18) v = w[co * 18 + hh * 9 + (n % 9)];
                else if (n == 18) { v = bias[co]; want_lo = hh != 0; }
                else if (X3 && n < 28) { v = w[co * 18 + hh * 9 + (n - 19)]; want_lo = true; }
                const __bf16 h = (__bf16)v;
                wa[cb][s][j] = want_lo ? (__bf16)(v - (float)h) : h;
            }
    const float act_pick = a <= 1.f ? __builtin_inff() : -__builtin_inff();

    const int segs_x = (W + 31) >> 5;
    const unsigned nseg = (unsigned)M * (unsigned)H * (unsigned)segs_x;
    const unsigned seg_step = gridDim.x * 4u;
    const int d_sx = (int)(seg_step % (unsigned)segs_x), d_y = (int)((seg_step / (unsigned)segs_x) % (unsigned)H);
    const int d_m = (int)(seg_step / ((unsigned)segs_x * (unsigned)H));
    auto advance = [&](int& m, int& y, int& sx) __attribute__((always_inline)) {
        sx += d_sx; y += d_y; m += d_m;
        if (sx >= segs_x) { sx -= segs_x; ++y; }
        if (y >= H) { y -= H; ++m; }
    };
    auto load_taps = [&](int m, int y, int sx, float (&v)[9]) __attribute__((always_inline)) {
        const int x = sx * 32 + r;
        const float* pb = hh ? in1 + (size_t)(m / rep1) * img_stride1 : in0 + (size_t)m * img_stride0;
#pragma unroll
        for (int dy = 0; dy < 3; ++dy) {
            const int gy = y + dy - 1;
            const bool oky = (unsigned)gy < (unsigned)H;
            const float* rp = pb + (size_t)(oky ? gy : 0) * W + (x - 1);
#pragma unroll
            for (int dx = 0; dx < 3; ++dx) v[dy * 3 + dx] = (oky && (unsigned)(x + dx - 1) < (unsigned)W) ? rp[dx] : 0.f;
        }
    };
    unsigned si = blockIdx.x * 4u + (unsigned)wave;
    int sx = (int)(si % (unsigned)segs_x), y = (int)((si / (unsigned)segs_x) % (unsigned)H), m = (int)(si / ((unsigned)segs_x * (unsigned)H));
    int nsx = sx, ny = y, nm = m;
    float vn[9];
    if (si < nseg) load_taps(m, y, sx, vn);
    for (; si < nseg; si += seg_step, sx = nsx, y = ny, m = nm) {
        __bf16 hi[9], lo[9];
#pragma unroll
        for (int t = 0; t < 9; ++t) {
            const __bf16 h = (__bf16)vn[t];
            hi[t] = h;
            lo[t] = (__bf16)(vn[t] - (float)h);
        }
        advance(nm, ny, nsx);
        if (si + seg_step < nseg) load_taps(nm, ny, nsx, vn);
        f32x16 acc[2];
#pragma unroll
        for (int cb = 0; cb < 2; ++cb)
#pragma unroll
            for (int e = 0; e < 16; ++e) acc[cb][e] = 0.f;
#pragma unroll
        for (int s = 0; s < NK; ++s) {
            bf16x8 bq;
#pragma unroll
            for (int j = 0; j < 8; ++j) {
                const int n = 8 * s + j;
                bq[j] = n < 9 ? hi[n] : (n < 18 ? lo[n - 9] : (n == 18 ? (__bf16)1.f : ((X3 && n < 28) ? hi[n - 19] : (__bf16)0.f)));
            }
            acc[0] = __builtin_amdgcn_mfma_f32_32x32x16_bf16(wa[0][s], bq, acc[0], 0, 0, 0);
            acc[1] = __builtin_amdgcn_mfma_f32_32x32x16_bf16(wa[1][s], bq, acc[1], 0, 0, 0);
        }
#pragma unroll
        for (int cb = 0; cb < 2; ++cb)
#pragma unroll
            for (int g = 0; g < 4; ++g) {
                const int co = cb * 32 + 8 * g + 4 * hh;
                f32x4 v;
#pragma unroll
                for (int j = 0; j < 4; ++j) {
                    const float t = acc[cb][4 * g + j];
                    v[j] = __builtin_amdgcn_fmed3f(t, a * t, act_pick);
                }
                if constexpr (X3) {
                    uint2 uh, ul;
                    split2_bf16(v[0], v[1], uh.x, ul.x);
                    split2_bf16(v[2], v[3], uh.y, ul.y);
                    *(uint2*)(stg + r * SROW + co * 2) = uh;
                    *(uint2*)(stg + 4 * 32 * SROW + r * SROW + co * 2) = ul;
                } else {
                    uint2 u;
                    u.x = pack2_bf16(v[0], v[1]);
                    u.y = pack2_bf16(v[2], v[3]);
                    *(uint2*)(stg + r * SROW + co * 2) = u;
                }
            }
        unsigned short* orow = out + (((size_t)m * H + y) * W + sx * 32) * 64;
#pragma unroll
        for (int i = 0; i < 4; ++i) {
            const int px = 8 * i + (lane >> 3), part = lane & 7;
            const u32x4 v = *(const u32x4*)(stg + px * SROW + part * 16);
            if (sx * 32 + px < W) __builtin_nontemporal_store(v, (u32x4*)(orow + (size_t)px * 64 + part * 8));
            if constexpr (X3) {
                const u32x4 vl = *(const u32x4*)(stg + 4 * 32 * SROW + px * SROW + part * 16);
                if (sx * 32 + px < W) __builtin_nontemporal_store(vl, (u32x4*)((unsigned char*)(orow + (size_t)px * 64 + part * 8) + out_lo));
            }
        }
    }
}

__global__ __launch_bounds__(256) void plane_mean_kernel(const float* __restrict__ x, float* __restrict__ mean, size_t hw) {
    const float* p = x + (size_t)blockIdx.x * hw;
    double s = 0.0;
    for (size_t i = threadIdx.x; i < hw; i += 256) s += (double)p[i];
    __shared__ double red[256];
    red[threadIdx.x] = s;
    __syncthreads();
    for (int st = 128; st > 0; st >>= 1) {
        if (threadIdx.x < st) red[threadIdx.x] += red[threadIdx.x + st];
        __syncthreads();
    }
    if (threadIdx.x == 0) mean[blockIdx.x] = (float)(red[0] / (double)hw);
}

template <bool LO>
__global__ __launch_bounds__(256) void planes_to_f32_kernel(const u32x4* __restrict__ hi, const u32x4* __restrict__ lo, float* __restrict__ out, size_t n8) {
    for (size_t i = (size_t)blockIdx.x * 256 + threadIdx.x; i < n8; i += (size_t)gridDim.x * 256) {
        const u32x4 h = hi[i];
        f32x4 a, b;
#pragma unroll
        for (int k = 0; k < 2; ++k) {
            a[2 * k] = __uint_as_float(h[k] << 16);
            a[2 * k + 1] = __uint_as_float(h[k] & 0xffff0000u);
            b[2 * k] = __uint_as_float(h[2 + k] << 16);
            b[2 * k + 1] = __uint_as_float(h[2 + k] & 0xffff0000u);
        }
        if constexpr (LO) {
            const u32x4 l = lo[i];
#pragma unroll
            for (int k = 0; k < 2; ++k) {
                a[2 * k] += __uint_as_float(l[k] << 16);
                a[2 * k + 1] += __uint_as_float(l[k] & 0xffff0000u);
                b[2 * k] += __uint_as_float(l[2 + k] << 16);
                b[2 * k + 1] += __uint_as_float(l[2 + k] & 0xffff0000u);
            }
        }
        *(f32x4*)(out + i * 8) = a;
        *(f32x4*)(out + i * 8 + 4) = b;
    }
}

template <bool LO>
__global__ __launch_bounds__(256) void f32_to_planes_kernel(const float* __restrict__ in, u32x4* __restrict__ hi, u32x4* __restrict__ lo, size_t n8) {
    for (size_t i = (size_t)blockIdx.x * 256 + threadIdx.x; i < n8; i += (size_t)gridDim.x * 256) {
        const f32x4 a = *(const f32x4*)(in + i * 8), b = *(const f32x4*)(in + i * 8 + 4);
        unsigned h[4], l[4];
        split2_bf16(a[0], a[1], h[0], l[0]); split2_bf16(a[2], a[3], h[1], l[1]);
        split2_bf16(b[0], b[1], h[2], l[2]); split2_bf16(b[2], b[3], h[3], l[3]);
        hi[i] = u32x4{h[0], h[1], h[2], h[3]};
        if constexpr (LO) lo[i] = u32x4{l[0], l[1], l[2], l[3]};
    }
}

}

int hrn_launch_median(const float* lrs, float* ref, int B, int V, int H, int W, hipStream_t stream) {
    const size_t hw = (size_t)H * W, total = (size_t)B * hw;
    const int blocks = (int)((total + 255) / 256 < 4096 ? (total + 255) / 256 : 4096);
    HrnProfScope prof("median9", 0.0, (double)total * 4 * ((V < 9 ? V : 9) + 1), stream);
    hipLaunchKernelGGL(median_kernel, dim3(blocks), dim3(256), 0, stream, lrs, ref, V, hw, total);
    HRN_LAUNCH_CHECK();
    return 0;
}

int hrn_launch_stem(int dt, const float* in0, size_t img_stride0, const float* in1, int rep1, size_t img_stride1,
                    const float* sub, const float* w, const float* bias, const float* slope, void* out,
                    int M, int H, int W, hipStream_t stream, size_t out_lo) {
    const size_t patches = (size_t)M * ((H + 3) / 4) * ((W + 31) / 32);
    const int blocks = (int)(patches < 16384 ? patches : 16384);
    const double px = (double)M * H * W;
    HrnProfScope prof(dt == HRN_BF16 ? "stem2x64_bf16" : dt == HRN_BF16X3 ? "stem2x64_bf16x3" : "stem2x64_f32", 2.0 * 18 * 64 * px, px * (4 + (double)M / rep1 / M * 4 + 64.0 * hrn_esize(dt)), stream);
    if ((dt == HRN_BF16 || dt == HRN_BF16X3) && sub == nullptr)
        HRN_CHECK((size_t)M * H * ((W + 31) / 32) < ((size_t)1 << 31), -2, "stem: %d images of %d x %d exceed the 32-bit segment count", M, H, W);
    if (dt == HRN_BF16 && sub == nullptr) {
        const size_t nseg = (size_t)M * H * ((W + 31) / 32);
        const int mblocks = (int)((nseg + 3) / 4 < 8192 ? (nseg + 3) / 4 : 8192);
        hipLaunchKernelGGL(stem_mfma_kernel<false>, dim3(mblocks), dim3(256), 0, stream, in0, in1, img_stride0, rep1, img_stride1, w, bias, slope,
                           (unsigned short*)out, M, H, W, (size_t)0);
    } else if (dt == HRN_BF16X3 && sub == nullptr) {
        HRN_CHECK(out_lo != 0, -2, "stem bf16x3: lo-plane offset missing");
        const size_t nseg = (size_t)M * H * ((W + 31) / 32);
        const int mblocks = (int)((nseg + 3) / 4 < 8192 ? (nseg + 3) / 4 : 8192);
        hipLaunchKernelGGL(stem_mfma_kernel<true>, dim3(mblocks), dim3(256), 0, stream, in0, in1, img_stride0, rep1, img_stride1, w, bias, slope,
                           (unsigned short*)out, M, H, W, out_lo);
    } else if (dt == HRN_BF16X3) {
        HRN_CHECK(out_lo != 0, -2, "stem bf16x3: lo-plane offset missing");
        hipLaunchKernelGGL(stem_kernel<HRN_BF16X3>, dim3(blocks), dim3(256), 0, stream, in0, in1, img_stride0, rep1, img_stride1, sub, w, bias, slope, out, M, H, W,
                           (const float*)nullptr, out_lo);
    } else if (dt == HRN_BF16)
        hipLaunchKernelGGL(stem_kernel<HRN_BF16>, dim3(blocks), dim3(256), 0, stream, in0, in1, img_stride0, rep1, img_stride1, sub, w, bias, slope, out, M, H, W,
                           (const float*)nullptr, (size_t)0);
    else
        hipLaunchKernelGGL(stem_kernel<HRN_F32>, dim3(blocks), dim3(256), 0, stream, in0, in1, img_stride0, rep1, img_stride1, sub, w, bias, slope, out, M, H, W,
                           (const float*)nullptr, (size_t)0);
    HRN_LAUNCH_CHECK();
    return 0;
}

int hrn_launch_stem_pre(int dt, const float* in0, size_t img_stride0, const float* in1, int rep1, size_t img_stride1, const float* w,
                        const float* bias, void* out, int M, int H, int W, const float* only_if_nonpos, hipStream_t stream) {
    const size_t patches = (size_t)M * ((H + 3) / 4) * ((W + 31) / 32);
    const int blocks = (int)(patches < 16384 ? patches : 16384);
    const size_t out_lo = dt == HRN_BF16X3 ? (size_t)M * H * W * 64 * 2 : 0;
    HRN_LAUNCH_ST(dt, stem_kernel, dim3(blocks), dim3(256), 0, stream, in0, in1, img_stride0, rep1, img_stride1, (const float*)nullptr, w, bias,
                  (const float*)nullptr, out, M, H, W, only_if_nonpos, out_lo);
    HRN_LAUNCH_CHECK();
    return 0;
}

int hrn_launch_planes_to_f32(const void* hi, size_t lo_off, float* out, size_t n, hipStream_t stream) {
    HRN_CHECK(n % 8 == 0 && lo_off % 16 == 0, -2, "planes_to_f32: %zu elements / lo offset %zu not aligned", n, lo_off);
    const size_t n8 = n / 8;
    const int blocks = (int)((n8 + 255) / 256 < 8192 ? (n8 + 255) / 256 : 8192);
    HrnProfScope prof("planes_to_f32", 0.0, (double)n * 8, stream);
    if (lo_off) hipLaunchKernelGGL(planes_to_f32_kernel<true>, dim3(blocks), dim3(256), 0, stream, (const u32x4*)hi, (const u32x4*)((const unsigned char*)hi + lo_off), out, n8);
    else hipLaunchKernelGGL(planes_to_f32_kernel<false>, dim3(blocks), dim3(256), 0, stream, (const u32x4*)hi, (const u32x4*)nullptr, out, n8);
    HRN_LAUNCH_CHECK();
    return 0;
}

int hrn_launch_f32_to_planes(const float* in, void* hi, size_t lo_off, size_t n, hipStream_t stream) {
    HRN_CHECK(n % 8 == 0 && lo_off % 16 == 0, -2, "f32_to_planes: %zu elements / lo offset %zu not aligned", n, lo_off);
    const size_t n8 = n / 8;
    const int blocks = (int)((n8 + 255) / 256 < 8192 ? (n8 + 255) / 256 : 8192);
    if (lo_off) hipLaunchKernelGGL(f32_to_planes_kernel<true>, dim3(blocks), dim3(256), 0, stream, in, (u32x4*)hi, (u32x4*)((unsigned char*)hi + lo_off), n8);
    else hipLaunchKernelGGL(f32_to_planes_kernel<false>, dim3(blocks), dim3(256), 0, stream, in, (u32x4*)hi, (u32x4*)nullptr, n8);
    HRN_LAUNCH_CHECK();
    return 0;
}

int hrn_launch_plane_mean(const float* x, float* mean, int planes, size_t hw, hipStream_t stream) {
    HrnProfScope prof("plane_mean", 0.0, (double)planes * hw * 4, stream);
    hipLaunchKernelGGL(plane_mean_kernel, dim3(planes), dim3(256), 0, stream, x, mean, hw);
    HRN_LAUNCH_CHECK();
    return 0;
}
```

Measured before the change: 2050.

## Fuse stem conv into first encoder residual block's conv3x3 kernels

With bf16, the stem conv (2->64 channels from the LR view and median reference) is now recomputed inside the first encoder conv3x3 r64 kernel, both as its input tile producer and as the residual for the second conv. This removes the stem kernel launch and the write and read of a 64-channel bf16 activation stack. The cost is recomputing stem MFMAs per halo tile and extra register pressure from the stem weight fragments and taps. An environment variable selects the route, with full fusion as the default.

```diff
diff --git a/highres-net_amd/hrnet_hip/csrc/api.hip b/highres-net_amd/hrnet_hip/csrc/api.hip
--- a/highres-net_amd/hrnet_hip/csrc/api.hip
+++ b/highres-net_amd/hrnet_hip/csrc/api.hip
@@ -54,25 +54,38 @@
     return 0;
 }
 
+int stem_fuse_default() {
+    static const int v = [] { const char* e = getenv("HRN_STEM_FUSE"); const int x = e ? atoi(e) : 2; return x < 0 ? 0 : x > 2 ? 2 : x; }();
+    return v;
+}
+
 int encoder_impl(const void* pk, int dt, int nl, const float* lrs, int B, int V, int H, int W,
-                 void* emb, void* ws, const HrnetWs& wl, hipStream_t s) {
+                 void* emb, void* ws, const HrnetWs& wl, hipStream_t s, int stem_route) {
     const HrnetLayout L = hrnet_layout(dt, nl, 3);
     const size_t hw = (size_t)H * W;
     float* ref = (float*)at(ws, wl.ref);
     void* bufA = at(ws, wl.buf_a);
     void* bufB = at(ws, wl.buf_b);
     int rc;
+    if (dt != HRN_BF16 || nl < 1 || !hrn_conv3x3_stem_fusable(B * V, H, W)) stem_route = 0;
     if ((rc = hrn_launch_median(lrs, ref, B, V, H, W, s))) return rc;
     const size_t lo = stack_lo(dt, B, V, H, W);
-    if ((rc = hrn_launch_stem(dt, lrs, hw, ref, V, hw, nullptr, (const float*)at(pk, L.stem_w), (const float*)at(pk, L.stem_b),
+    if (stem_route < 2 &&
+        (rc = hrn_launch_stem(dt, lrs, hw, ref, V, hw, nullptr, (const float*)at(pk, L.stem_w), (const float*)at(pk, L.stem_b),
                               (const float*)at(pk, L.stem_a), bufA, B * V, H, W, s, lo))) return rc;
+    auto stem_desc = [&](ConvParams& c) {
+        c.stem_in0 = lrs; c.stem_stride0 = hw; c.stem_in1 = ref; c.stem_rep1 = V; c.stem_stride1 = hw;
+        c.stem_w = (const float*)at(pk, L.stem_w); c.stem_b = (const float*)at(pk, L.stem_b); c.stem_a = (const float*)at(pk, L.stem_a);
+    };
     for (int l = 0; l < nl; ++l) {
         ConvParams p = conv_base(B * V, H, W);
         p.in = bufA; p.out = bufB; p.in_lo = p.out_lo = lo;
+        if (l == 0 && stem_route == 2) { p.in = nullptr; p.stem_in = 1; stem_desc(p); }
         p.wpk = at(pk, L.enc_w[2 * l]); p.bias = (const float*)at(pk, L.enc_b[2 * l]); p.slope = (const float*)at(pk, L.enc_a[2 * l]);
         if ((rc = hrn_launch_conv3x3(dt, 64, 64, p, s, false))) return rc;
         ConvParams q = conv_base(B * V, H, W);
         q.in = bufB; q.out = bufA; q.res = bufA; q.res_mode = 1; q.in_lo = q.out_lo = q.res_lo = lo;
+        if (l == 0 && stem_route >= 1) { q.res = nullptr; q.res_mode = 4; stem_desc(q); }
         q.wpk = at(pk, L.enc_w[2 * l + 1]); q.bias = (const float*)at(pk, L.enc_b[2 * l + 1]); q.slope = (const float*)at(pk, L.enc_a[2 * l + 1]);
         if ((rc = hrn_launch_conv3x3(dt, 64, 64, q, s, false))) return rc;
     }
@@ -148,6 +161,17 @@
 
 }
 
+int hrn_encoder_forward_route(int stem_route, const void* packed, int dt, int nl, const float* lrs, int B, int V, int H, int W,
+                              void* emb, void* ws, size_t ws_bytes, hipStream_t stream) {
+    int rc;
+    if ((rc = check_common(dt, nl, B, V, H, W))) return rc;
+    HRN_CHECK(stem_route >= 0 && stem_route <= 2, -2, "hrn_encoder_forward_route: route %d", stem_route);
+    HRN_CHECK(packed && lrs && emb && ws, -2, "hrn_encoder_forward: null argument");
+    const HrnetWs wl = hrnet_ws(dt, B, V, H, W);
+    HRN_CHECK(ws_bytes >= wl.total, -3, "hrn_encoder_forward: workspace too small (%zu < %zu)", ws_bytes, wl.total);
+    return encoder_impl(packed, dt, nl, lrs, B, V, H, W, emb, ws, wl, stream, stem_route);
+}
+
 extern "C" {
 
 int hrn_version(void) { return HRN_ABI_VERSION; }
@@ -201,12 +225,7 @@
 
 int hrn_encoder_forward(const void* packed, int dt, int nl, const float* lrs, int B, int V, int H, int W,
                         void* emb, void* ws, size_t ws_bytes, void* stream) {
-    int rc;
-    if ((rc = check_common(dt, nl, B, V, H, W))) return rc;
-    HRN_CHECK(packed && lrs && emb && ws, -2, "hrn_encoder_forward: null argument");
-    const HrnetWs wl = hrnet_ws(dt, B, V, H, W);
-    HRN_CHECK(ws_bytes >= wl.total, -3, "hrn_encoder_forward: workspace too small (%zu < %zu)", ws_bytes, wl.total);
-    return encoder_impl(packed, dt, nl, lrs, B, V, H, W, emb, ws, wl, (hipStream_t)stream);
+    return hrn_encoder_forward_route(stem_fuse_default(), packed, dt, nl, lrs, B, V, H, W, emb, ws, ws_bytes, (hipStream_t)stream);
 }
 
 int hrn_fuse_forward(const void* packed, int dt, int nl, int alpha_residual, void* emb, const float* alphas,
@@ -236,7 +255,7 @@
     hipStream_t s = (hipStream_t)stream;
     void* emb = at(ws, wl.emb);
     void* fused = at(ws, wl.fused);
-    if ((rc = encoder_impl(packed, dt, nl, lrs, B, V, H, W, emb, ws, wl, s))) return rc;
+    if ((rc = encoder_impl(packed, dt, nl, lrs, B, V, H, W, emb, ws, wl, s, stem_fuse_default()))) return rc;
     if ((rc = fuse_impl(packed, dt, nl, alpha_residual, emb, alphas, B, V, H, W, fused, ws, wl, s))) return rc;
     return decoder_impl(packed, dt, nl, scale, fused, B, H, W, sr, s);
 }
diff --git a/highres-net_amd/hrnet_hip/csrc/conv3x3.h b/highres-net_amd/hrnet_hip/csrc/conv3x3.h
--- a/highres-net_amd/hrnet_hip/csrc/conv3x3.h
+++ b/highres-net_amd/hrnet_hip/csrc/conv3x3.h
@@ -24,6 +24,15 @@
     const float* scale;
     size_t in_lo, stack_lo, out_lo, res_lo;
     const float* only_if_nonpos;
+    const float* stem_in0;
+    size_t stem_stride0;
+    const float* stem_in1;
+    int stem_rep1;
+    size_t stem_stride1;
+    const float* stem_w;
+    const float* stem_b;
+    const float* stem_a;
+    int stem_in;
 };
 
 static inline size_t conv_packed_elems(int cin, int cout) { return (size_t)cin * cout * 9; }
@@ -31,6 +40,8 @@
 int hrn_launch_conv3x3(int dt, int cin, int cout, const ConvParams& p, hipStream_t stream, bool general_only);
 
 int hrn_launch_conv3x3_r64(const ConvParams& p, hipStream_t stream);
+bool hrn_conv3x3_r64_fits(int M, int H, int W);
+bool hrn_conv3x3_stem_fusable(int M, int H, int W);
 
 int hrn_launch_conv3x3_v6(int cin, int cout, const ConvParams& p, hipStream_t stream);
 
diff --git a/highres-net_amd/hrnet_hip/csrc/conv3x3.hip b/highres-net_amd/hrnet_hip/csrc/conv3x3.hip
--- a/highres-net_amd/hrnet_hip/csrc/conv3x3.hip
+++ b/highres-net_amd/hrnet_hip/csrc/conv3x3.hip
@@ -334,16 +334,30 @@
 
 }
 
+static int conv_r64_enabled() {
+    static const int r64 = [] { const char* e = getenv("HRN_CONV_R64"); return e ? atoi(e) : 1; }();
+    return r64;
+}
+
+bool hrn_conv3x3_stem_fusable(int M, int H, int W) { return conv_r64_enabled() && hrn_conv3x3_r64_fits(M, H, W); }
+
 int hrn_launch_conv3x3(int dt, int cin, int cout, const ConvParams& p, hipStream_t stream, bool general_only) {
     HRN_CHECK(p.M > 0 && p.H > 0 && p.W > 0, -2, "conv3x3: empty problem M=%d H=%d W=%d", p.M, p.H, p.W);
     HRN_CHECK(!p.in_pair || (cin == 128 && p.pair_h > 0 && p.stack), -2, "conv3x3: pair input needs cin=128 and a pair descriptor");
     HRN_CHECK(p.res_mode != 2 || (p.pair_h > 0 && p.stack && cout == 128), -2, "conv3x3: res_mode 2 needs a pair descriptor and cout=128");
-    HRN_CHECK(p.in_pair || p.in, -2, "conv3x3: null input");
+    HRN_CHECK(p.in_pair || p.in || p.stem_in, -2, "conv3x3: null input");
     HRN_CHECK(p.res_mode != 3 || p.out_h > 0, -2, "conv3x3: res_mode 3 needs slot output");
     HRN_CHECK(!(general_only && dt == HRN_BF16X3), -2, "conv3x3: bf16x3 has no general kernel");
+    if (p.res_mode == 4 || p.stem_in) {
+        HRN_CHECK(dt == HRN_BF16 && cin == 64 && cout == 64 && !general_only && hrn_conv3x3_stem_fusable(p.M, p.H, p.W), -2,
+                  "conv3x3: res_mode 4 / stem_in need the bf16 64 -> 64 resident-weights kernel (dt=%d %d->%d M=%d H=%d W=%d)", dt, cin, cout, p.M, p.H, p.W);
+        const int rc = hrn_launch_conv3x3_r64(p, stream);
+        HRN_CHECK(rc != -100, -2, "conv3x3: conv3x3_r64 declined a layer with stem fields");
+        return rc;
+    }
     if (dt == HRN_BF16X3) return hrn_launch_conv3x3_v6x3(cin, cout, p, stream);
     if (dt == HRN_BF16 && !p.scale && !p.relu && !general_only) {
-        static const int r64 = [] { const char* e = getenv("HRN_CONV_R64"); return e ? atoi(e) : 1; }();
+        const int r64 = conv_r64_enabled();
         static const int v6 = [] { const char* e = getenv("HRN_CONV_V6"); return e ? atoi(e) : 1; }();
         if (cin == 64 && cout == 64 && r64) { const int rc = hrn_launch_conv3x3_r64(p, stream); if (rc != -100) return rc; }
         if ((cin == 128 || cout == 128) && v6) { const int rc = hrn_launch_conv3x3_v6(cin, cout, p, stream); if (rc != -100) return rc; }
diff --git a/highres-net_amd/hrnet_hip/csrc/conv3x3_r64.hip b/highres-net_amd/hrnet_hip/csrc/conv3x3_r64.hip
--- a/highres-net_amd/hrnet_hip/csrc/conv3x3_r64.hip
+++ b/highres-net_amd/hrnet_hip/csrc/conv3x3_r64.hip
@@ -1,5 +1,6 @@
 #include <type_traits>
 #include "conv3x3.h"
+#include "stem_segment.h"
 
 namespace {
 
@@ -23,8 +24,9 @@
 
 __device__ __attribute__((aligned(16))) unsigned hrn_r64_zero16[4];
 
-template <bool RES>
+template <bool RES, int STEM>
 __global__ __launch_bounds__(512, 2) void conv3x3_r64_kernel(const ConvParams p) {
+    static_assert(STEM == 0 || (STEM == 1 && RES) || (STEM == 2 && !RES), "stem variant");
     if (p.only_if_nonpos && p.only_if_nonpos[0] > 0.f) return;
     extern __shared__ __attribute__((aligned(16))) unsigned char smem[];
     unsigned char* w_lds = smem;
@@ -63,8 +65,72 @@
         if (tid < 64) bias_lds[tid] = p.bias[tid];
     }
 
+    bf16x8 swa[2][3];
+    float stem_a = 1.f, stem_pick = 0.f;
+    if constexpr (STEM != 0) {
+        stem_weight_frags<3>(p.stem_w, p.stem_b, r, hh, swa);
+        stem_a = p.stem_a ? p.stem_a[0] : 1.f;
+        stem_pick = stem_act_pick(stem_a);
+    }
+    auto stem_plane = [&](unsigned m) __attribute__((always_inline)) {
+        const float* pv = p.stem_in0 + (size_t)m * p.stem_stride0;
+        const float* pr = p.stem_in1 + (size_t)(m / (unsigned)p.stem_rep1) * p.stem_stride1;
+        asm volatile("" : "+s"(pv), "+s"(pr));
+        return hh ? pr : pv;
+    };
+    float ptap[3][9];
+    auto produce_load = [&](unsigned m, unsigned t) __attribute__((always_inline)) {
+        const int ty = t / tiles_x;
+        const int y0 = ty * CONV_TILE_H, x0 = (t - ty * tiles_x) * CONV_TILE_W;
+        const float* pl = stem_plane(m);
+#pragma unroll
+        for (int jj = 0; jj < 3; ++jj) {
+            const int j = tw + 4 * jj;
+            if (j < 11) {
+                const int hp = 32 * j + r;
+                const int py = hp / HALO_W, px = hp - py * HALO_W;
+                const int gy = y0 - 1 + py, gx = x0 - 1 + px;
+#pragma unroll
+                for (int dy = 0; dy < 3; ++dy) {
+                    const int yy = gy + dy - 1;
+                    const bool oky = (unsigned)yy < (unsigned)H;
+                    const float* rp = pl + (long)(oky ? yy : 0) * W + (gx - 1);
+#pragma unroll
+                    for (int dx = 0; dx < 3; ++dx) ptap[jj][dy * 3 + dx] = (oky && (unsigned)(gx + dx - 1) < (unsigned)W) ? rp[dx] : 0.f;
+                }
+            }
+        }
+    };
+    auto produce_write = [&](unsigned t) __attribute__((always_inline)) {
+        const int ty = t / tiles_x;
+        const int y0 = ty * CONV_TILE_H, x0 = (t - ty * tiles_x) * CONV_TILE_W;
+#pragma unroll
+        for (int jj = 0; jj < 3; ++jj) {
+            const int j = tw + 4 * jj;
+            if (j < 11) {
+                const int hp = 32 * j + r;
+                const int py = hp / HALO_W, px = hp - py * HALO_W;
+                const bool inimg = (unsigned)(y0 - 1 + py) < (unsigned)H && (unsigned)(x0 - 1 + px) < (unsigned)W;
+                f32x16 sx[2];
+                stem_segment(swa, ptap[jj], stem_a, stem_pick, sx);
+                unsigned char* dst = in_lds + hp * 128 + hh * 8;
+                const int sw = (hp >> 1) & 7;
+                if (hp < HALO_H * HALO_W) {
+#pragma unroll
+                    for (int cb = 0; cb < 2; ++cb)
+#pragma unroll
+                        for (int g = 0; g < 4; ++g) {
+                            u32x2 u = {pack2_bf16(sx[cb][4 * g], sx[cb][4 * g + 1]), pack2_bf16(sx[cb][4 * g + 2], sx[cb][4 * g + 3])};
+                            if (!inimg) u = u32x2{0u, 0u};
+                            *(u32x2*)(dst + (((4 * cb + g) ^ sw) << 4)) = u;
+                        }
+                }
+            }
+        }
+    };
+
     unsigned voff[11], cm_lo = 0, cm_hi = 0;
-    if (!RES) {
+    if (!RES && STEM != 2) {
 #pragma unroll
         for (int jj = 0; jj < 11; ++jj) {
             const int j = tw + 4 * jj;
@@ -78,6 +144,7 @@
     }
     unsigned pend_F = 0;
     auto issue = [&](unsigned m, unsigned t) __attribute__((always_inline)) {
+        if constexpr (STEM == 2) { produce_write(t); return; }
         const int ty = t / tiles_x;
         const int y0 = ty * CONV_TILE_H, x0 = (t - ty * tiles_x) * CONV_TILE_W;
         const unsigned char* base = (const unsigned char*)p.in + (size_t)m * hw * 128;
@@ -119,7 +186,7 @@
         __builtin_amdgcn_sched_barrier(0);
     };
     auto fix_borders = [&]() __attribute__((always_inline)) {
-        if (!RES && pend_F) {
+        if (!RES && STEM != 2 && pend_F) {
             const unsigned fm = pend_F * 0x11111111u;
             const unsigned hit_lo = cm_lo & fm, hit_hi = cm_hi & fm;
             const u32x4 z = {0u, 0u, 0u, 0u};
@@ -214,10 +281,24 @@
 
     u32x4 resv[2][4];
     float res_alpha = 1.f;
+    float rtap[4][3];
     auto fetch_residual = [&]() __attribute__((always_inline)) {
         const int m = (int)cur_m;
         const int ty = cur_t / tiles_x;
         const int y0 = ty * CONV_TILE_H, x0 = (cur_t - ty * tiles_x) * CONV_TILE_W;
+        if constexpr (STEM == 1) {
+            const float* pl = stem_plane((unsigned)m);
+            const int x = x0 + r;
+#pragma unroll
+            for (int row = 0; row < 4; ++row) {
+                const int gy = y0 + 2 * tw + row - 1;
+                const bool oky = (unsigned)gy < (unsigned)H;
+                const float* rp = pl + (long)(oky ? gy : 0) * W + (x - 1);
+#pragma unroll
+                for (int dx = 0; dx < 3; ++dx) rtap[row][dx] = (oky && (unsigned)(x + dx - 1) < (unsigned)W) ? rp[dx] : 0.f;
+            }
+            return;
+        }
         const unsigned char* rbase = (const unsigned char*)p.res + (size_t)m * hw * 128;
         if (p.res_mode == 3) {
             const int ob = m / p.out_h, oi = m - ob * p.out_h;
@@ -232,6 +313,30 @@
                 const int gxj = x0 + (r & ~3) + j, gxjc = gxj < W ? gxj : W - 1;
                 resv[pb][j] = __builtin_nontemporal_load((const u32x4*)(rbase + (unsigned)((gyc * W + gxjc) * 128 + hh * 64 + (r & 3) * 16)));
             }
+        }
+    };
+
+    unsigned sres[2][2][4][2];
+    auto stem_residual = [&]() __attribute__((always_inline)) {
+        __bf16 rhi[4][3], rlo[4][3];
+#pragma unroll
+        for (int row = 0; row < 4; ++row)
+#pragma unroll
+            for (int dx = 0; dx < 3; ++dx) stem_split_tap(rtap[row][dx], rhi[row][dx], rlo[row][dx]);
+#pragma unroll
+        for (int pb = 0; pb < 2; ++pb) {
+            __bf16 hi[9], lo[9];
+#pragma unroll
+            for (int t = 0; t < 9; ++t) { hi[t] = rhi[pb + t / 3][t % 3]; lo[t] = rlo[pb + t / 3][t % 3]; }
+            f32x16 sx[2];
+            stem_segment_mma<3>(swa, hi, lo, sx);
+#pragma unroll
+            for (int cb = 0; cb < 2; ++cb)
+#pragma unroll
+                for (int g = 0; g < 4; ++g)
+#pragma unroll
+                    for (int h = 0; h < 2; ++h)
+                        sres[pb][cb][g][h] = pack2_bf16(stem_prelu(sx[cb][4 * g + 2 * h], stem_a, stem_pick), stem_prelu(sx[cb][4 * g + 2 * h + 1], stem_a, stem_pick));
         }
     };
 
@@ -245,7 +350,8 @@
         int ob = 0, oi = 0;
         if (p.out_h > 0) { ob = m / p.out_h; oi = m - ob * p.out_h; oimg = (size_t)ob * p.out_vs + oi; }
         unsigned char* outp = (unsigned char*)p.out + (oimg * hw + (size_t)y0 * W + x0) * 128;
-        if (RES) {
+        if constexpr (STEM == 1) {
+        } else if (RES) {
 #pragma unroll
             for (int pb = 0; pb < 2; ++pb)
 #pragma unroll
@@ -259,7 +365,7 @@
         for (int pb = 0; pb < 2; ++pb) {
             const int gy = y0 + 2 * tw + pb;
             u32x4 uu[4];
-            if (RES) quad_transpose(resv[pb], (lane & 1) != 0, (lane & 2) != 0);
+            if (RES && STEM == 0) quad_transpose(resv[pb], (lane & 1) != 0, (lane & 2) != 0);
 #pragma unroll
             for (int g = 0; g < 4; ++g) {
                 float xa[4], xb[4];
@@ -272,8 +378,15 @@
 #pragma unroll
                     for (int j = 0; j < 4; ++j) { xa[j] = xa[j] >= 0.f ? xa[j] : slope * xa[j]; xb[j] = xb[j] >= 0.f ? xb[j] : slope * xb[j]; }
                 }
+                if constexpr (STEM == 1) {
+                    const unsigned qa0 = sres[pb][0][g][0], qa1 = sres[pb][0][g][1], qb0 = sres[pb][1][g][0], qb1 = sres[pb][1][g][1];
+                    xa[0] += __uint_as_float(qa0 << 16); xa[1] += __uint_as_float(qa0 & 0xffff0000u);
+                    xa[2] += __uint_as_float(qa1 << 16); xa[3] += __uint_as_float(qa1 & 0xffff0000u);
+                    xb[0] += __uint_as_float(qb0 << 16); xb[1] += __uint_as_float(qb0 & 0xffff0000u);
+                    xb[2] += __uint_as_float(qb1 << 16); xb[3] += __uint_as_float(qb1 & 0xffff0000u);
+                }
                 u32x4 u;
-                if (RES) {
+                if (RES && STEM == 0) {
                     float v[8];
 #pragma unroll
                     for (int j = 0; j < 4; ++j) {
@@ -311,13 +424,15 @@
         else epilogue(std::integral_constant<int, 2>{});
         {
             const int nst = 4 * ((y0 + 2 * tw < H) + (y0 + 2 * tw + 1 < H));
-            if (nst == 8) asm volatile("s_waitcnt vmcnt(8)" ::: "memory");
+            if constexpr (STEM == 2) {}
+            else if (nst == 8) asm volatile("s_waitcnt vmcnt(8)" ::: "memory");
             else if (nst == 4) asm volatile("s_waitcnt vmcnt(4)" ::: "memory");
             else asm volatile("s_waitcnt vmcnt(0)" ::: "memory");
         }
         fix_borders();
     };
 
+    if constexpr (STEM == 2) { if (nmine > 0) produce_load(cur_m, cur_t); }
     if (nmine > 0) issue(cur_m, cur_t);
     asm volatile("s_waitcnt vmcnt(0)" ::: "memory");
     fix_borders();
@@ -328,7 +443,18 @@
         if (q >= 0) {
             const int k = q >> 1;
             if (k < nmine) {
-                if ((q & 1) == 0) { if (RES) fetch_residual(); multiply(); }
+                if ((q & 1) == 0) {
+                    if (RES) fetch_residual();
+                    multiply();
+                    if constexpr (STEM == 1) stem_residual();
+                    if constexpr (STEM == 2) {
+                        if (k + 1 < nmine) {
+                            unsigned nt = cur_t + step_t, nm = cur_m + step_m;
+                            if (nt >= tiles) { nt -= tiles; ++nm; }
+                            produce_load(nm, nt);
+                        }
+                    }
+                }
                 else finish(k + 1 < nmine);
             }
         }
@@ -337,10 +463,10 @@
 }
 
 
-template <bool RES>
+template <bool RES, int STEM>
 int launch_r64(const ConvParams& p, long grid, hipStream_t stream) {
-    { const int rc_lds = hrn_allow_lds((const void*)conv3x3_r64_kernel<RES>, LDS_BYTES); if (rc_lds) return rc_lds; }
-    hipLaunchKernelGGL(conv3x3_r64_kernel<RES>, dim3((unsigned)grid), dim3(512), LDS_BYTES, stream, p);
+    { const int rc_lds = hrn_allow_lds((const void*)conv3x3_r64_kernel<RES, STEM>, LDS_BYTES); if (rc_lds) return rc_lds; }
+    hipLaunchKernelGGL((conv3x3_r64_kernel<RES, STEM>), dim3((unsigned)grid), dim3(512), LDS_BYTES, stream, p);
     HRN_LAUNCH_CHECK();
     return 0;
 }
@@ -353,12 +479,25 @@
     const long tiles = (long)((p.W + CONV_TILE_W - 1) / CONV_TILE_W) * ((p.H + CONV_TILE_H - 1) / CONV_TILE_H);
     const long total = tiles * p.M;
     HRN_CHECK(total > 0, -2, "conv3x3_r64: bad tile count %ld", total);
-    if (total >= (1L << 30) || (long)p.H * p.W * 128 >= (1L << 31)) return -100;
+    if (!hrn_conv3x3_r64_fits(p.M, p.H, p.W)) return -100;
+    const bool sres = p.res_mode == 4, sin = p.stem_in != 0;
+    if (sres || sin)
+        HRN_CHECK(!(sres && sin) && p.stem_in0 && p.stem_in1 && p.stem_w && p.stem_b && p.stem_rep1 > 0 && (sin ? p.res_mode == 0 : true), -2,
+                  "conv3x3_r64: incomplete stem descriptor (res_mode %d, stem_in %d)", p.res_mode, p.stem_in);
+    HRN_CHECK(sin || p.in, -2, "conv3x3_r64: null input");
     long grid = hrn_device_cus();
     if (total < grid) grid = total;
     if (grid >= 8) grid &= ~7L;
     const double px = (double)p.M * p.H * p.W;
-    HrnProfScope prof(p.res_mode ? "conv3x3_bf16_64x64+res" : "conv3x3_bf16_64x64", 2.0 * 64 * 64 * 9 * px,
-                      px * 2 * (64 + 64 + (p.res_mode ? 64 : 0)), stream);
-    return p.res_mode ? launch_r64<true>(p, grid, stream) : launch_r64<false>(p, grid, stream);
-}
+    HrnProfScope prof(sin ? "conv3x3_bf16_64x64+stemin" : sres ? "conv3x3_bf16_64x64+stemres" : p.res_mode ? "conv3x3_bf16_64x64+res" : "conv3x3_bf16_64x64",
+                      (2.0 * 64 * 64 * 9 + (sres || sin ? 2.0 * 18 * 64 : 0.0)) * px,
+                      sin ? px * (8 + 128) : sres ? px * (8 + 256) : px * 2 * (64 + 64 + (p.res_mode ? 64 : 0)), stream);
+    if (sin) return launch_r64<false, 2>(p, grid, stream);
+    if (sres) return launch_r64<true, 1>(p, grid, stream);
+    return p.res_mode ? launch_r64<true, 0>(p, grid, stream) : launch_r64<false, 0>(p, grid, stream);
+}
+
+bool hrn_conv3x3_r64_fits(int M, int H, int W) {
+    const long tiles = (long)((W + CONV_TILE_W - 1) / CONV_TILE_W) * ((H + CONV_TILE_H - 1) / CONV_TILE_H);
+    return tiles * M < (1L << 30) && (long)H * W * 128 < (1L << 31);
+}
diff --git a/highres-net_amd/hrnet_hip/csrc/kernels.h b/highres-net_amd/hrnet_hip/csrc/kernels.h
--- a/highres-net_amd/hrnet_hip/csrc/kernels.h
+++ b/highres-net_amd/hrnet_hip/csrc/kernels.h
@@ -1,6 +1,9 @@
 #pragma once
 #include "common.h"
 #include "conv3x3.h"
+
+int hrn_encoder_forward_route(int stem_route, const void* packed, int dt, int nl, const float* lrs, int B, int V, int H, int W,
+                              void* emb, void* ws, size_t ws_bytes, hipStream_t stream);
 
 int hrn_launch_median(const float* lrs, float* ref, int B, int V, int H, int W, hipStream_t stream);
 int hrn_launch_stem(int dt, const float* in0, size_t img_stride0, const float* in1, int rep1, size_t img_stride1,
diff --git a/highres-net_amd/hrnet_hip/csrc/stem.hip b/highres-net_amd/hrnet_hip/csrc/stem.hip
--- a/highres-net_amd/hrnet_hip/csrc/stem.hip
+++ b/highres-net_amd/hrnet_hip/csrc/stem.hip
@@ -1,4 +1,5 @@
 #include "kernels.h"
+#include "stem_segment.h"
 
 namespace {
 
@@ -143,22 +144,8 @@
     unsigned char* stg = stg_all + wave * 32 * SROW;
 
     bf16x8 wa[2][NK];
-#pragma unroll
-    for (int cb = 0; cb < 2; ++cb)
-#pragma unroll
-        for (int s = 0; s < NK; ++s)
-#pragma unroll
-            for (int j = 0; j < 8; ++j) {
-                const int n = 8 * s + j, co = cb * 32 + r;
-                float v = 0.f;
-                bool want_lo = false;
-                if (n < 18) v = w[co * 18 + hh * 9 + (n % 9)];
-                else if (n == 18) { v = bias[co]; want_lo = hh != 0; }
-                else if (X3 && n < 28) { v = w[co * 18 + hh * 9 + (n - 19)]; want_lo = true; }
-                const __bf16 h = (__bf16)v;
-                wa[cb][s][j] = want_lo ? (__bf16)(v - (float)h) : h;
-            }
-    const float act_pick = a <= 1.f ? __builtin_inff() : -__builtin_inff();
+    stem_weight_frags<NK>(w, bias, r, hh, wa);
+    const float act_pick = stem_act_pick(a);
 
     const int segs_x = (W + 31) >> 5;
     const unsigned nseg = (unsigned)M * (unsigned)H * (unsigned)segs_x;
@@ -190,29 +177,11 @@
     for (; si < nseg; si += seg_step, sx = nsx, y = ny, m = nm) {
         __bf16 hi[9], lo[9];
 #pragma unroll
-        for (int t = 0; t < 9; ++t) {
-            const __bf16 h = (__bf16)vn[t];
-            hi[t] = h;
-            lo[t] = (__bf16)(vn[t] - (float)h);
-        }
+        for (int t = 0; t < 9; ++t) stem_split_tap(vn[t], hi[t], lo[t]);
         advance(nm, ny, nsx);
         if (si + seg_step < nseg) load_taps(nm, ny, nsx, vn);
         f32x16 acc[2];
-#pragma unroll
-        for (int cb = 0; cb < 2; ++cb)
-#pragma unroll
-            for (int e = 0; e < 16; ++e) acc[cb][e] = 0.f;
-#pragma unroll
-        for (int s = 0; s < NK; ++s) {
-            bf16x8 bq;
-#pragma unroll
-            for (int j = 0; j < 8; ++j) {
-                const int n = 8 * s + j;
-                bq[j] = n < 9 ? hi[n] : (n < 18 ? lo[n - 9] : (n == 18 ? (__bf16)1.f : ((X3 && n < 28) ? hi[n - 19] : (__bf16)0.f)));
-            }
-            acc[0] = __builtin_amdgcn_mfma_f32_32x32x16_bf16(wa[0][s], bq, acc[0], 0, 0, 0);
-            acc[1] = __builtin_amdgcn_mfma_f32_32x32x16_bf16(wa[1][s], bq, acc[1], 0, 0, 0);
-        }
+        stem_segment_mma<NK>(wa, hi, lo, acc);
 #pragma unroll
         for (int cb = 0; cb < 2; ++cb)
 #pragma unroll
@@ -222,7 +191,7 @@
 #pragma unroll
                 for (int j = 0; j < 4; ++j) {
                     const float t = acc[cb][4 * g + j];
-                    v[j] = __builtin_amdgcn_fmed3f(t, a * t, act_pick);
+                    v[j] = stem_prelu(t, a, act_pick);
                 }
                 if constexpr (X3) {
                     uint2 uh, ul;
diff --git a/highres-net_amd/hrnet_hip/csrc/stem_segment.h b/highres-net_amd/hrnet_hip/csrc/stem_segment.h
--- /dev/null
+++ b/highres-net_amd/hrnet_hip/csrc/stem_segment.h
@@ -0,0 +1,61 @@
+#pragma once
+#include "common.h"
+
+template <int NK>
+__device__ __forceinline__ void stem_weight_frags(const float* __restrict__ w, const float* __restrict__ bias, int r, int hh, bf16x8 (&wa)[2][NK]) {
+#pragma unroll
+    for (int cb = 0; cb < 2; ++cb)
+#pragma unroll
+        for (int s = 0; s < NK; ++s)
+#pragma unroll
+            for (int j = 0; j < 8; ++j) {
+                const int n = 8 * s + j, co = cb * 32 + r;
+                float v = 0.f;
+                bool want_lo = false;
+                if (n < 18) v = w[co * 18 + hh * 9 + (n % 9)];
+                else if (n == 18) { v = bias[co]; want_lo = hh != 0; }
+                else if (NK == 4 && n < 28) { v = w[co * 18 + hh * 9 + (n - 19)]; want_lo = true; }
+                const __bf16 h = (__bf16)v;
+                wa[cb][s][j] = want_lo ? (__bf16)(v - (float)h) : h;
+            }
+}
+
+__device__ __forceinline__ float stem_act_pick(float a) { return a <= 1.f ? __builtin_inff() : -__builtin_inff(); }
+
+__device__ __forceinline__ void stem_split_tap(float v, __bf16& hi, __bf16& lo) {
+    const __bf16 h = (__bf16)v;
+    hi = h;
+    lo = (__bf16)(v - (float)h);
+}
+
+template <int NK>
+__device__ __forceinline__ void stem_segment_mma(const bf16x8 (&wa)[2][NK], const __bf16 (&hi)[9], const __bf16 (&lo)[9], f32x16 (&acc)[2]) {
+#pragma unroll
+    for (int cb = 0; cb < 2; ++cb)
+#pragma unroll
+        for (int e = 0; e < 16; ++e) acc[cb][e] = 0.f;
+#pragma unroll
+    for (int s = 0; s < NK; ++s) {
+        bf16x8 bq;
+#pragma unroll
+        for (int j = 0; j < 8; ++j) {
+            const int n = 8 * s + j;
+            bq[j] = n < 9 ? hi[n] : (n < 18 ? lo[n - 9] : (n == 18 ? (__bf16)1.f : ((NK == 4 && n < 28) ? hi[n - 19] : (__bf16)0.f)));
+        }
+        acc[0] = __builtin_amdgcn_mfma_f32_32x32x16_bf16(wa[0][s], bq, acc[0], 0, 0, 0);
+        acc[1] = __builtin_amdgcn_mfma_f32_32x32x16_bf16(wa[1][s], bq, acc[1], 0, 0, 0);
+    }
+}
+
+__device__ __forceinline__ float stem_prelu(float t, float a, float act_pick) { return __builtin_amdgcn_fmed3f(t, a * t, act_pick); }
+
+__device__ __forceinline__ void stem_segment(const bf16x8 (&wa)[2][3], const float (&taps)[9], float a, float act_pick, f32x16 (&out)[2]) {
+    __bf16 hi[9], lo[9];
+#pragma unroll
+    for (int t = 0; t < 9; ++t) stem_split_tap(taps[t], hi[t], lo[t]);
+    stem_segment_mma<3>(wa, hi, lo, out);
+#pragma unroll
+    for (int cb = 0; cb < 2; ++cb)
+#pragma unroll
+        for (int e = 0; e < 16; ++e) out[cb][e] = stem_prelu(out[cb][e], a, act_pick);
+}
```

New measurement: 2070 (median of 6 runs). No clear change (+1.0%).
